# Borx25/CPU-Raytracing-experiments

Hardware: NVIDIA B200
Metric: Mrays/s (higher is better)
Workload: dtype f32

## Files before the change

__graft_entry__.py:

```python
import os
import subprocess
import sys

ROOT = os.path.dirname(os.path.abspath(__file__))
PKG = os.path.join(ROOT, "cpu-raytracing-experiments_b200")
CSRC = os.path.join(PKG, "csrc")
NVCC = os.environ.get("NVCC", "/usr/local/cuda/bin/nvcc")

NVCC_FLAGS = ["-gencode", "arch=compute_100a,code=sm_100a", "-lineinfo", "-O3", "-std=c++17", "-fmad=false",
              "-Xcompiler", "-fPIC,-ffp-contract=off,-O2", "-shared"]


def _newer(target, sources):
    if not os.path.exists(target):
        return True
    t = os.path.getmtime(target)
    return any(os.path.getmtime(s) > t for s in sources)


def build_lib(force=False):
    srcs = [os.path.join(CSRC, f) for f in ("b2r.cu", "b2r_host.cpp")]
    deps = srcs + [os.path.join(CSRC, f) for f in ("b2r_device.cuh", "b2r_shade.h", "b2r_math.h", "b2r_host.h")] + [os.path.join(ROOT, "include", "b2r.h")]
    out = os.path.join(PKG, "libb2r.so")
    if force or _newer(out, deps):
        subprocess.check_call([NVCC] + NVCC_FLAGS + srcs + ["-o", out])
    return out


def build_hostcheck(force=False):
    src = os.path.join(ROOT, "tests", "hostcheck", "hostcheck.cpp")
    out = os.path.join(ROOT, "tests", "hostcheck", "libhostcheck.so")
    cam = os.path.join(ROOT, "tests", "hostcheck", "mirror_camera.cpp")
    deps = [src, cam] + [os.path.join(CSRC, f) for f in ("b2r_host.cpp", "b2r_shade.h", "b2r_math.h", "b2r_host.h")] + [os.path.join(PKG, "host", f) for f in ("Camera.hpp", "Core.hpp")]
    if force or _newer(out, deps):
        subprocess.check_call(["g++", "-std=c++17", "-O2", "-ffp-contract=off", "-mavx2", "-mfma", "-fPIC", "-shared",
                               "-I/usr/local/cuda/include", "-I", CSRC, "-I", os.path.join(PKG, "host"), src, cam, os.path.join(CSRC, "b2r_host.cpp"), "-o", out])
    return out


def build_oracle():
    sys.path.insert(0, os.path.join(ROOT, "oracle"))
    import oracle_py
    srcs = [os.path.join(ROOT, "oracle", f) for f in ("oracle.cpp", "oracle_math.hpp")]
    force = any(_newer(os.path.join(ROOT, "oracle", n), srcs) for n in ("liboracle.so", "liboracle_fast.so"))
    oracle_py.build(force=force)


def build_refbinding(force=False):
    if not os.path.isdir("/root/reference"):
        return None
    d = os.path.join(ROOT, "tests", "refbinding"); out = os.path.join(d, "refbinding")
    deps = [os.path.join(d, "refbinding.cpp"), os.path.join(d, "build.sh"), os.path.join(ROOT, "include", "b2r_reference_binding.hpp"),
            os.path.join(ROOT, "include", "b2r.h"), os.path.join(PKG, "libb2r.so")]
    if force or _newer(out, deps):
        subprocess.check_call([os.path.join(d, "build.sh")], stdout=subprocess.DEVNULL)
    return out


def build():
    build_lib()
    build_oracle()
    build_hostcheck()
    build_refbinding()
    sys.path.insert(0, PKG)
    import b2r
    L = b2r.lib()
    assert L.b2r_abi_version() == 1
    missing = [s for s in b2r.ABI_SYMBOLS if not hasattr(L, s)]
    assert not missing, missing


def smoke():
    import numpy as np
    build()
    sys.path.insert(0, PKG); sys.path.insert(0, os.path.join(ROOT, "oracle"))
    import b2r, scenes, oracle_py
    W, H, MB, K = 256, 144, 8, 5
    sc = scenes.default_scene()
    r = b2r.Renderer(sc, W, H, max_bounces=MB, buckets=K)
    r.Accumulate(K)
    assert r.Render()
    o = oracle_py.Oracle(W, H, max_bounces=MB, K=K); o.set_scene(sc); o.accumulate(K)
    rc, ref = o.render()
    gb, ob = r.buckets_host(), o.buckets()
    rel = np.abs(gb - ob) / np.maximum(np.abs(ob), 1e-6)
    divergent = float((rel > 1e-4).any(axis=(0, 1)).mean())
    rmse = float(np.sqrt(np.mean((r.framebuffer[..., :3] - ref[..., :3]) ** 2)))
    print(f"smoke: brute default scene {W}x{H} K={K}: divergent pixel fraction {divergent:.2e}, bit-exact {bool((gb.view(np.uint32) == ob.view(np.uint32)).all())}, framebuffer RMSE {rmse:.3e}; counters {r.counters()}")
    assert divergent < 1e-3 and rmse < 1e-3
    if oracle_py.have_reference_renderer():
        rr = oracle_py.ReferenceRenderer(sc, W, H, MB); rr.accumulate(K); rb = rr.buckets(); _, rframe = rr.render(); rr.close()
        relr = np.abs(gb - rb) / np.maximum(np.abs(rb), 1e-6)
        div_r = float((relr > 1e-4).any(axis=(0, 1)).mean())
        rmse_r = float(np.sqrt(np.mean((r.framebuffer[..., :3] - rframe[..., :3]) ** 2)))
        print(f"smoke: against THE REFERENCE's Renderer::Accumulate/Render (oracle/_ref/librefrenderer.so): divergent pixel fraction {div_r:.2e}, framebuffer RMSE {rmse_r:.3e}")
        assert div_r < 5e-3 and rmse_r < 5e-3
    sc2 = scenes.random_scene(600, light_every=40)
    r2 = b2r.Renderer(sc2, 128, 64, max_bounces=6, buckets=1, flags=b2r.FLAG_FORCE_BVH)
    r2.Accumulate(2)
    o2 = oracle_py.Oracle(128, 64, max_bounces=6, K=1); o2.set_scene(sc2); o2.accumulate(2)
    g2, ob2 = r2.buckets_host(), o2.buckets()
    rel2 = np.abs(g2 - ob2) / np.maximum(np.abs(ob2), 1e-6)
    div2 = float((rel2 > 1e-4).any(axis=(0, 1)).mean())
    print(f"smoke: BVH pipeline random600 128x64: divergent pixel fraction {div2:.2e}")
    assert div2 < 5e-3
    geo = sc2["geometry"].copy(); rs = np.random.RandomState(1)
    geo["position"] += (rs.uniform(-0.5, 0.5, (len(geo), 3)) * np.sqrt(geo["radius_sq"])[:, None]).astype(np.float32)
    q = r2.RefitScene(geo); r2.ResetAccumulator(); r2.Accumulate(2)
    sc3 = scenes.Scene(sc2); sc3["geometry"] = geo
    o3 = oracle_py.Oracle(128, 64, max_bounces=6, K=1); o3.set_scene(sc3); o3.accumulate(2)
    g3, ob3 = r2.buckets_host(), o3.buckets()
    div3 = float(((np.abs(g3 - ob3) / np.maximum(np.abs(ob3), 1e-6)) > 1e-4).any(axis=(0, 1)).mean())
    print(f"smoke: after b2r_refit_scene (every sphere moved, tree quality ratio {q:.3f}): divergent pixel fraction {div3:.2e}")
    assert div3 < 5e-3
    r3 = b2r.Renderer(sc3, 128, 64, max_bounces=6, buckets=1, flags=b2r.FLAG_FORCE_BVH | b2r.FLAG_GPU_TREE | b2r.FLAG_GPU_SAH)
    r3.Accumulate(2)
    same = r3.buckets_host().tobytes() == g3.tobytes()
    print(f"smoke: device-built sweep tree ({len(r3.wide_nodes()[0])} wide nodes): buckets bit-identical to the host-built tree's: {same}")
    assert same
# ... 9 lines not shown
```

cpu-raytracing-experiments_b200/b2r.py:

```python
import ctypes as C
import os

import numpy as np

try:
    from . import scenes as _scenes
except ImportError:
    import scenes as _scenes

_HERE = os.path.dirname(os.path.abspath(__file__))
LIB_PATH = os.environ.get("B2R_LIB_PATH", os.path.join(_HERE, "libb2r.so"))

FLAG_FORCE_BRUTE, FLAG_FORCE_BVH, FLAG_NO_MIS, FLAG_COUNT_TESTS, FLAG_NO_GRAPH, FLAG_REFERENCE_TREE, FLAG_REFERENCE_EXACT, FLAG_NO_SPECULATION, FLAG_GPU_TREE = 1, 2, 4, 8, 16, 32, 64, 128, 256
FLAG_GPU_SAH = 1024
FLAG_GPU_SAH3 = 2048
FLAG_GGX = 512
FLAG_DIELECTRIC = 4096
TAP_CLOSEST, TAP_SHADOW, TAP_PACKET = 0, 1, 2
OK, ERR_ARG, ERR_CUDA, ERR_STATE, ERR_NO_LIGHTS, ERR_BVH, NOT_READY = 0, -1, -2, -3, -4, -5, 1
KERNEL_KINDS = ["generate", "bounce_brute", "intersect_closest", "shade", "intersect_shadow", "accumulate", "resolve"]
COUNTER_NAMES = ["extension_rays", "shadow_rays", "shaded_hits", "terminated", "dropped", "sphere_tests", "box_tests", "launches", "radiance_events", "reserved"]

ABI_SYMBOLS = [
    "b2r_bvh_build", "b2r_bvh_build_ex", "b2r_find_lights", "b2r_camera_lookat", "b2r_camera_ray", "b2r_create", "b2r_destroy", "b2r_resize", "b2r_reset", "b2r_set_stream",
    "b2r_sync", "b2r_upload_scene", "b2r_refit_scene", "b2r_set_camera", "b2r_set_lens", "b2r_accumulate", "b2r_resolve", "b2r_resolve_async", "b2r_resolve_device", "b2r_frame_wait", "b2r_resolve_from", "b2r_ipc_export_buckets", "b2r_ipc_open_peers", "b2r_ipc_close", "b2r_resolve_peers", "b2r_team_export", "b2r_team_open", "b2r_team_resolve", "b2r_team_error", "b2r_team_close", "b2r_host_register", "b2r_host_unregister", "b2r_get_accumulations", "b2r_set_accumulations",
    "b2r_read_buckets", "b2r_write_buckets", "b2r_save_checkpoint", "b2r_load_checkpoint", "b2r_device_buckets", "b2r_device_framebuffer", "b2r_read_counters", "b2r_reset_counters", "b2r_read_bounce_counts",
    "b2r_read_kernel_times", "b2r_set_flags", "b2r_generate_rays", "b2r_trace_closest", "b2r_trace_shadow", "b2r_trace_kernel", "b2r_read_wide_nodes", "b2r_read_link_tables", "b2r_get_origin_box",
    "b2r_write_hdr", "b2r_read_hdr", "b2r_last_error", "b2r_abi_version",
]


class B2RError(RuntimeError):
    def __init__(self, code, text):
        super().__init__(f"libb2r error {code}: {text}")
        self.code = code


class Config(C.Structure):
    _fields_ = [("width", C.c_uint32), ("height", C.c_uint32), ("max_bounces", C.c_uint32), ("buckets", C.c_uint32), ("flags", C.c_uint32),
                ("device", C.c_int32), ("bucket_first", C.c_uint32), ("bucket_stride", C.c_uint32), ("samples_in_flight", C.c_uint32)]


_lib = None


def lib():
    global _lib
    if _lib is None:
        if not os.path.exists(LIB_PATH):
            raise B2RError(ERR_STATE, f"{LIB_PATH} not built - run `python -c 'import __graft_entry__ as g; g.build()'`")
        L = C.CDLL(LIB_PATH)
        vp, u32, i32, f32 = C.c_void_p, C.c_uint32, C.c_int32, C.c_float
        sig = {
            "b2r_bvh_build": [vp, u32, vp, vp, vp, vp], "b2r_bvh_build_ex": [vp, u32, u32, f32, vp, vp, vp, vp], "b2r_find_lights": [vp, u32, vp, u32, vp, vp],
            "b2r_camera_lookat": [vp, vp, u32, u32, f32, f32, vp], "b2r_camera_ray": [vp, vp, f32, f32, f32, i32, i32, vp, vp, vp], "b2r_create": [vp, vp], "b2r_resize": [vp, u32, u32], "b2r_reset": [vp],
            "b2r_set_stream": [vp, vp], "b2r_sync": [vp],
            "b2r_upload_scene": [vp, vp, vp, u32, u32, vp, u32, vp, u32, vp, u32, vp, vp, i32, i32],
            "b2r_refit_scene": [vp, vp, u32, vp, u32, vp, u32, vp, u32, vp],
            "b2r_set_camera": [vp, vp, vp, f32, f32, f32, f32], "b2r_set_lens": [vp, f32, f32], "b2r_accumulate": [vp, u32], "b2r_resolve": [vp, vp, C.c_int], "b2r_resolve_async": [vp, vp, C.c_int], "b2r_resolve_device": [vp, C.c_int], "b2r_frame_wait": [vp], "b2r_resolve_from": [vp, vp, vp, C.c_int], "b2r_ipc_export_buckets": [vp, vp], "b2r_ipc_open_peers": [vp, vp, u32, u32], "b2r_ipc_close": [vp], "b2r_resolve_peers": [vp, vp, C.c_int], "b2r_team_export": [vp, vp], "b2r_team_open": [vp, vp, u32, u32], "b2r_team_resolve": [vp, vp, C.c_int, C.c_int], "b2r_team_error": [vp, vp], "b2r_team_close": [vp],
            "b2r_host_register": [vp, C.c_size_t], "b2r_host_unregister": [vp], "b2r_get_accumulations": [vp, vp], "b2r_set_accumulations": [vp, u32], "b2r_read_buckets": [vp, vp], "b2r_write_buckets": [vp, vp],
            "b2r_device_buckets": [vp, vp, vp], "b2r_device_framebuffer": [vp, vp, vp], "b2r_read_counters": [vp, vp], "b2r_reset_counters": [vp], "b2r_read_bounce_counts": [vp, vp, vp, u32],
            "b2r_read_kernel_times": [vp, vp, vp, C.c_int], "b2r_set_flags": [vp, u32], "b2r_generate_rays": [vp, u32, vp],
            "b2r_save_checkpoint": [vp, C.c_char_p], "b2r_load_checkpoint": [vp, C.c_char_p], "b2r_write_hdr": [C.c_char_p, vp, u32, u32], "b2r_read_hdr": [C.c_char_p, vp, vp, vp], "b2r_trace_closest": [vp, vp, u32, vp, vp], "b2r_trace_shadow": [vp, vp, vp, u32, vp], "b2r_trace_kernel": [vp, C.c_int, vp, vp, vp, vp, u32, u32, vp, vp, vp], "b2r_read_wide_nodes": [vp, vp, vp, vp], "b2r_read_link_tables": [vp, vp, vp], "b2r_get_origin_box": [vp, vp],
        }
        for name, args in sig.items():
            fn = getattr(L, name); fn.argtypes = args; fn.restype = C.c_int
        L.b2r_destroy.argtypes = [vp]; L.b2r_destroy.restype = None
        L.b2r_last_error.restype = C.c_char_p; L.b2r_abi_version.restype = C.c_int
        _lib = L
    return _lib


def _check(rc):
    if rc < 0:
        raise B2RError(rc, lib().b2r_last_error().decode())
    return rc


def _ptr(a):
    return C.c_void_p(a.ctypes.data) if a is not None else None


def build_bvh(geometry, log_cluster_size=0, cost_ratio=1.0):
    geo = np.ascontiguousarray(geometry, dtype=_scenes.SPHERE_DTYPE); n = len(geo)
    nodes = np.zeros(max(1, 2 * n - 1), _scenes.NODE_DTYPE); prims = np.zeros(n, _scenes.SPHERE_DTYPE); ids = np.zeros(n, np.uint32)
    nn = C.c_uint32(0)
    _check(lib().b2r_bvh_build_ex(_ptr(geo), n, log_cluster_size, cost_ratio, _ptr(nodes), _ptr(prims), _ptr(ids), C.addressof(nn)))
    return nodes[:nn.value], prims, ids


def find_lights(geometry, material):
    geo = np.ascontiguousarray(geometry, dtype=_scenes.SPHERE_DTYPE); mat = np.ascontiguousarray(material, dtype=_scenes.MATERIAL_DTYPE)
    out = np.zeros(len(geo), np.int32); n = C.c_uint32(0)
    _check(lib().b2r_find_lights(_ptr(geo), len(geo), _ptr(mat), len(mat), _ptr(out), C.addressof(n)))
    return out[:n.value].copy()


def camera_lookat(eye, direction, width, height, focal_length, exposure=1.0):
    out = np.zeros(11, np.float32)
    e = np.asarray(eye, np.float32); d = np.asarray(direction, np.float32)
    _check(lib().b2r_camera_lookat(_ptr(e), _ptr(d), width, height, focal_length, exposure, _ptr(out)))
    return out


class PreparedScene:

    def __init__(self, scene, width, height):
        self.scene = scene
        self.geometry = np.ascontiguousarray(scene["geometry"], dtype=_scenes.SPHERE_DTYPE)
        self.material = np.ascontiguousarray(scene["material"], dtype=_scenes.MATERIAL_DTYPE)
        self.nodes, self.prims, self.prim_ids = build_bvh(self.geometry)
        self.lights = find_lights(self.geometry, self.material)
        self.ambient = np.asarray(scene["ambient"], np.float32)
        self.hdri = None if scene.get("hdri") is None else np.ascontiguousarray(scene["hdri"], np.float32)
        self.set_view(width, height)

    def set_view(self, width, height):
        cam = self.scene["camera"]
        self.camera = camera_lookat(cam["eye"], cam["dir"], width, height, cam["focal_length"], cam["exposure"])


class Renderer:

    TileRoot = 16

    @staticmethod
    def RequiredTiling():
        return 16

    def __init__(self, scene, width, height, max_bounces=16, buckets=5, flags=0, device=0, bucket_first=0, bucket_stride=0,
                 samples_in_flight=0, stream=None):
        self._h = C.c_void_p(None)
        cfg = Config(width, height, max_bounces, buckets, flags, device, bucket_first, bucket_stride, samples_in_flight)
        _check(lib().b2r_create(C.byref(self._h), C.byref(cfg)))
        self.width, self.height, self.max_bounces, self.buckets, self.flags = width, height, max_bounces, buckets, flags
        self.h_tiles, self.v_tiles = width // 16, height // 16
        self.framebuffer = np.zeros((height, width, 4), np.float32)
        if stream is not None:
            _check(lib().b2r_set_stream(self._h, C.c_void_p(stream)))
        self.scene = None
        if scene is not None:
            self.SetScene(scene)

    def close(self):
        if getattr(self, "_h", None) and self._h.value:
            lib().b2r_destroy(self._h); self._h = C.c_void_p(None)
# ... 101 lines not shown
        return _check(lib().b2r_team_resolve(self._h, _ptr(dst), 1 if tonemap else 0, 1 if use_async else 0)) == OK

    def team_error(self):
        v = C.c_uint32(0); _check(lib().b2r_team_error(self._h, C.byref(v))); return v.value

    def GetFrame(self):
        return self.framebuffer

    def sync(self):
        _check(lib().b2r_sync(self._h))

    def buckets_host(self):
        out = np.empty((self.buckets, 3, self.width * self.height), np.float32); _check(lib().b2r_read_buckets(self._h, _ptr(out))); return out

    def write_buckets(self, arr):
        a = np.ascontiguousarray(arr, np.float32); _check(lib().b2r_write_buckets(self._h, _ptr(a)))

    def SaveCheckpoint(self, path):
        _check(lib().b2r_save_checkpoint(self._h, str(path).encode()))

    def LoadCheckpoint(self, path):
        _check(lib().b2r_load_checkpoint(self._h, str(path).encode()))

    def device_buckets(self):
        p = C.c_void_p(None); n = C.c_size_t(0); _check(lib().b2r_device_buckets(self._h, C.byref(p), C.byref(n))); return p.value, n.value

    def device_framebuffer(self):
        p = C.c_void_p(None); n = C.c_size_t(0); _check(lib().b2r_device_framebuffer(self._h, C.byref(p), C.byref(n))); return p.value, n.value

    def counters(self):
        out = (C.c_uint64 * 10)(); _check(lib().b2r_read_counters(self._h, out)); return dict(zip(COUNTER_NAMES, out[:]))

    def bounce_counts(self):
        n = self.max_bounces + 1; a = np.zeros(n, np.uint32); b = np.zeros(n, np.uint32)
        _check(lib().b2r_read_bounce_counts(self._h, _ptr(a), _ptr(b), n)); return a, b

    def reset_counters(self):
        _check(lib().b2r_reset_counters(self._h))

    def kernel_times(self, reset=True):
        ms = (C.c_double * 8)(); n = (C.c_uint64 * 8)(); _check(lib().b2r_read_kernel_times(self._h, ms, n, 1 if reset else 0))
        return {k: (ms[i], n[i]) for i, k in enumerate(KERNEL_KINDS)}

    def set_flags(self, flags):
        _check(lib().b2r_set_flags(self._h, flags)); self.flags = flags

    def generate_rays(self, acc):
        out = np.empty((self.width * self.height, 6), np.float32); _check(lib().b2r_generate_rays(self._h, acc, _ptr(out))); return out

    def trace_closest(self, rays):
        r = np.ascontiguousarray(rays, np.float32); n = len(r); t = np.empty(n, np.float32); p = np.empty(n, np.int32)
        _check(lib().b2r_trace_closest(self._h, _ptr(r), n, _ptr(t), _ptr(p))); return t, p

    def trace_shadow(self, rays, tfar):
        r = np.ascontiguousarray(rays, np.float32); tf = np.ascontiguousarray(tfar, np.float32); n = len(r); o = np.empty(n, np.uint8)
        _check(lib().b2r_trace_shadow(self._h, _ptr(r), _ptr(tf), n, _ptr(o))); return o

    def trace_kernel_closest(self, rays, tail=None):
        r = np.ascontiguousarray(rays, np.float32); n = len(r); t = np.empty(n, np.float32); p = np.empty(n, np.int32)
        tl = None if tail is None else np.ascontiguousarray(tail, np.uint8)
        _check(lib().b2r_trace_kernel(self._h, TAP_CLOSEST, _ptr(r), None, None, _ptr(tl), n, 0, _ptr(t), _ptr(p), None)); return t, p

    def trace_kernel_shadow(self, rays, tfar, origin_prim):
        r = np.ascontiguousarray(rays, np.float32); tf = np.ascontiguousarray(tfar, np.float32); op = np.ascontiguousarray(origin_prim, np.int32)
        n = len(r); o = np.empty(n, np.uint8)
        _check(lib().b2r_trace_kernel(self._h, TAP_SHADOW, _ptr(r), _ptr(tf), _ptr(op), None, n, 0, None, None, _ptr(o))); return o

    def trace_kernel_packet(self, acc):
        n = self.width * self.height; t = np.empty(n, np.float32); p = np.empty(n, np.int32)
        _check(lib().b2r_trace_kernel(self._h, TAP_PACKET, None, None, None, None, n, acc, _ptr(t), _ptr(p), None)); return t, p

    def link_tables(self):
        n = C.c_uint32(0); _check(lib().b2r_read_wide_nodes(self._h, None, C.byref(n), None))
        parent = np.empty(n.value, np.uint32); leaf = np.empty(len(self.scene.prims), np.uint32)
        _check(lib().b2r_read_link_tables(self._h, _ptr(parent), _ptr(leaf))); return parent, leaf

    def wide_nodes(self):
        n = C.c_uint32(0); ms = C.c_uint32(0)
        _check(lib().b2r_read_wide_nodes(self._h, None, C.byref(n), C.byref(ms)))
        out = np.zeros((n.value, 4, 8), np.float32)
        _check(lib().b2r_read_wide_nodes(self._h, _ptr(out), C.byref(n), C.byref(ms)))
        return out, ms.value

    def origin_box(self):
        out = np.zeros(6, np.float32); _check(lib().b2r_get_origin_box(self._h, _ptr(out))); return out


def host_register(arr):
    _check(lib().b2r_host_register(_ptr(arr), arr.nbytes))


def host_unregister(arr):
    _check(lib().b2r_host_unregister(_ptr(arr)))


def write_hdr(path, rgba):
    a = np.ascontiguousarray(rgba, np.float32)
    _check(lib().b2r_write_hdr(str(path).encode(), _ptr(a), a.shape[1], a.shape[0]))


def read_hdr(path):
    w, h = C.c_int32(0), C.c_int32(0)
    if lib().b2r_read_hdr(str(path).encode(), None, C.byref(w), C.byref(h)) != OK:
        raise B2RError(ERR_ARG, f"{path}: not a Radiance .hdr stb_image would load")
    out = np.empty((h.value, w.value, 4), np.float32)
    if lib().b2r_read_hdr(str(path).encode(), _ptr(out), C.byref(w), C.byref(h)) != OK:
        raise B2RError(ERR_ARG, f"{path}: corrupt or truncated .hdr")
    return out


def tile_to_raster(buf, width, height):
    ht, vt = width // 16, height // 16
    a = np.asarray(buf).reshape(buf.shape[:-1] + (vt, ht, 16, 16))
    return np.moveaxis(a, -2, -3).reshape(buf.shape[:-1] + (height, width))
```

cpu-raytracing-experiments_b200/csrc/b2r.cu:

```cuda
#include "b2r_device.cuh"

#include <cub/device/device_radix_sort.cuh>
#include <cub/device/device_scan.cuh>

#include <algorithm>
#include <cstdio>
#include <cstdlib>
#include <cstring>
#include <string>
#include <vector>

using namespace b2r;

namespace {

thread_local std::string g_error;
int fail(int code, const std::string& what) { g_error = what; return code; }
constexpr const char* kDielInvalid = "B2R_FLAG_DIELECTRIC: a material has a non-finite transmission, or is dielectric (max(transmission) > 0) with a transmission outside [0, 1] or 1 + IOR_minus_one not finite or < 1";
#define CU(expr) do { cudaError_t e_ = (expr); if (e_ != cudaSuccess) return fail(B2R_ERR_CUDA, std::string(#expr) + ": " + cudaGetErrorString(e_)); } while (0)

enum KernelKind { KK_GENERATE = 0, KK_BRUTE, KK_CLOSEST, KK_SHADE, KK_SHADOW, KK_ACCUMULATE, KK_RESOLVE, KK_COUNT };

constexpr uint32_t kMaxLanes = 4;
struct BatchArgs {
	uint32_t n; uint32_t acc[kMaxSlots]; unsigned long long fold = ~0ull; CameraParams cam; LensParams lens{0.0f, 0.0f};
	uint32_t lanes = 0, lane_slots = 0, n_lane[kMaxLanes] = {0, 0, 0, 0};
	uint32_t slot_of(uint32_t i) const {
		if (lanes == 0u) return i;
		uint32_t j = 0; while (j + 1u < lanes && i >= n_lane[j]) { i -= n_lane[j]; j++; }
		return j * lane_slots + i;
	}
};
__global__ void k_set_batch(BatchDev* dst, const BatchArgs a) {
	if (threadIdx.x == 0) { dst[0].n_slots = a.n; dst[0].fold = a.fold; dst[0].cam = a.cam; dst[0].lens = a.lens; }
	if (threadIdx.x < a.n) dst[0].acc[threadIdx.x] = a.acc[threadIdx.x];
	for (uint32_t j = 0; j < kMaxLanes; j++) {
		const uint32_t nj = j < a.lanes ? a.n_lane[j] : 0u;
		if (threadIdx.x == 0) { dst[1 + j].n_slots = nj; dst[1 + j].fold = 0ull; dst[1 + j].cam = a.cam; dst[1 + j].lens = a.lens; }
		if (threadIdx.x < nj) dst[1 + j].acc[threadIdx.x] = a.acc[j * a.lane_slots + threadIdx.x];
	}
}

template <typename T> int dev_alloc(T** p, size_t count) {
	if (*p) { cudaFree(*p); *p = nullptr; }
	if (count == 0) count = 1;
	CU(cudaMalloc(reinterpret_cast<void**>(p), count * sizeof(T)));
	return B2R_OK;
}
template <typename T> int dev_reserve(T** p, size_t* capacity, size_t count) {
	if (count == 0) count = 1;
	if (*p && *capacity >= count) return B2R_OK;
	if (*p) { cudaFree(*p); *p = nullptr; *capacity = 0; }
	CU(cudaMalloc(reinterpret_cast<void**>(p), count * sizeof(T)));
	*capacity = count;
	return B2R_OK;
}
template <typename T> void dev_free(T** p) { if (*p) { cudaFree(*p); *p = nullptr; } }

#define B2R_PACKED_TABLES(X) X(float4, prims, LEN_PRIMS) X(int32_t, prim_mat, LEN_PRIMS) X(float4, mat_albedo, LEN_MAT) X(float4, mat_emission, LEN_MAT) \
                             X(float4, mat_f0, LEN_MAT) X(float4, mat_diel, LEN_MAT) X(float4, light_sphere, LEN_LIGHTS) X(float4, light_emit, LEN_LIGHTS)
#define B2R_SCENE_TABLES(X) B2R_PACKED_TABLES(X) X(WideNode, wide, LEN_WIDE) X(uint32_t, parent, LEN_WIDE) X(uint32_t, leaf_node, LEN_PRIMS) X(float4, hdri, LEN_TEXELS)
enum TableLen { LEN_PRIMS = 0, LEN_MAT, LEN_LIGHTS, LEN_WIDE, LEN_TEXELS, LEN_COUNT };
struct SceneTables {
	template <typename T> struct Table { T* p = nullptr; size_t cap = 0; };
#define X(T, name, len) Table<T> name;
	B2R_SCENE_TABLES(X)
#undef X
	template <typename F, typename... S> static int for_each(F&& f, S&... sets) {
		int rc = B2R_OK;
#define X(T, name, len) if (rc == B2R_OK) rc = f(len, sets.name...);
		B2R_SCENE_TABLES(X)
#undef X
		return rc;
	}
};
void free_tables(SceneTables& t) { SceneTables::for_each([](int, auto& x) -> int { dev_free(&x.p); x.cap = 0; return B2R_OK; }, t); }
void bind_tables(Params& p, const SceneTables& t, bool sky) {
	SceneDev& s = p.scene;
	s.prims = t.prims.p; s.prim_mat = t.prim_mat.p; s.mat_albedo = t.mat_albedo.p; s.mat_emission = t.mat_emission.p; s.mat_f0 = t.mat_f0.p;
	s.light_sphere = t.light_sphere.p; s.light_emit = t.light_emit.p; s.wide = t.wide.p; s.parent = t.parent.p; s.leaf_node = t.leaf_node.p;
	s.hdri = sky ? t.hdri.p : nullptr;
	p.mat_diel = t.mat_diel.p;
}

}

struct b2r_ctx {
	b2r_config cfg{};
	cudaStream_t stream = nullptr, own_stream = nullptr;
	unsigned char* h_stage = nullptr; size_t stage_bytes = 0; cudaEvent_t ev_stage = nullptr; bool stage_busy = false;
	cudaStream_t copy_stream = nullptr; cudaEvent_t ev_resolved = nullptr, ev_copied = nullptr; bool copy_pending = false;
	bool have_scene = false, have_camera = false, use_bvh = false;
	uint32_t accumulations = 0;
	uint32_t slots = 8;
	int sm_count = 0;
	SceneTables tables;
	bool scene_diel_valid = true;
	WideBvh wide_host; uint64_t wide_key = 0; std::vector<unsigned char> wide_blob; bool have_wide = false;
	uint32_t n_wide = 0;
	bool gpu_tree = false; uint32_t *d_mkey[2] = {nullptr, nullptr}, *d_midx[2] = {nullptr, nullptr}; size_t cap_mkey = 0; uint8_t* d_sort_tmp = nullptr; size_t cap_sort_tmp = 0; uint8_t* d_sweep = nullptr; size_t cap_sweep = 0;
	std::vector<b2r_sphere> lazy_prims, lazy_geom; double* d_cost_base = nullptr;
	std::vector<uint32_t> cur_geom_of_prim;
	uint32_t* d_remap = nullptr; size_t cap_remap = 0;
	uint8_t* d_trace = nullptr; size_t cap_trace = 0;
	uint8_t* d_tap = nullptr; size_t cap_tap = 0;
	bool wide_refit = false; double* d_cost = nullptr;
	OriginBox obox{}; bool obox_valid = false; float sph_lo[3] = {0, 0, 0}, sph_hi[3] = {0, 0, 0}; float cam_pos[3] = {0, 0, 0};
	LensParams lens{0.0f, 0.0f};
	float4 *d_A[2] = {nullptr, nullptr}, *d_B[2] = {nullptr, nullptr}, *d_SA = nullptr, *d_SB = nullptr, *d_fb = nullptr;
	float *d_T[2] = {nullptr, nullptr}, *d_SL = nullptr, *d_rad = nullptr, *d_acc = nullptr;
	uint8_t *d_ex_slot[2] = {nullptr, nullptr}, *d_ex_key = nullptr; uint16_t* d_ex_act[2] = {nullptr, nullptr}; uint32_t* d_ex_next = nullptr;
	float2* d_H = nullptr; uint32_t* d_SS = nullptr;
	uint32_t* d_counts = nullptr; size_t counts_bytes = 0;
	unsigned long long* d_stats = nullptr;
	BatchDev* d_batch = nullptr;
	Params params{};
	int grid_brute_first_exact = 0, grid_brute_exact = 0;
	int grid_brute_first_ggx = 0, grid_brute_ggx = 0, grid_brute_finish_ggx = 0, grid_shade_ggx = 0;
	int grid_brute_first = 0, grid_brute = 0, grid_closest = 0, grid_shade = 0, grid_shadow = 0, grid_stream = 0, grid_packet = 0, grid_brute_finish = 0; bool packet_primary = true;
	int grid_brute_first_lens = 0, grid_brute_first_ggx_lens = 0, grid_packet_lens = 0;
	int grid_diel_brute_first[2][2] = {{0, 0}, {0, 0}}, grid_diel_brute[2] = {0, 0}, grid_diel_finish[2] = {0, 0}, grid_diel_shade[2] = {0, 0};
	cudaGraphExec_t graph_exec = nullptr; bool graph_valid = false;
	cudaGraphExec_t lane_exec[kMaxLanes + 1] = {nullptr, nullptr, nullptr, nullptr, nullptr}; bool lane_valid[kMaxLanes + 1] = {false, false, false, false, false};
	bool idle = true;
	uint32_t lanes_max = 2; bool lanes_forced = false;
	cudaStream_t lane_stream[kMaxLanes] = {nullptr, nullptr, nullptr, nullptr}; cudaEvent_t ev_fork = nullptr, ev_join[kMaxLanes] = {nullptr, nullptr, nullptr, nullptr};
	float lane_grid_frac = 1.0f;
	uint64_t graph_launches = 0, lane_launches[kMaxLanes + 1] = {0, 0, 0, 0, 0};
	struct Side {
		cudaStream_t stream = nullptr, lane_stream[kMaxLanes] = {nullptr, nullptr, nullptr, nullptr};
		cudaEvent_t ev_traced = nullptr, ev_folded = nullptr, ev_sync = nullptr, ev_fork = nullptr, ev_join[kMaxLanes] = {nullptr, nullptr, nullptr, nullptr};
		bool folded_valid = false; uint64_t epoch = ~0ull;
		SceneTables tables;
		bool have_copy = false, refreshed_valid = false; uint64_t scene_version = ~0ull; cudaEvent_t ev_refreshed = nullptr;
		cudaGraphExec_t exec[kMaxLanes + 1] = {nullptr, nullptr, nullptr, nullptr, nullptr}; bool valid[kMaxLanes + 1] = {false, false, false, false, false}; uint64_t launches[kMaxLanes + 1] = {0, 0, 0, 0, 0};
	} side[2];
	uint32_t sides = 2, next_side = 0, last_side = 0, spec_side = 0, counts_first = 0;
	uint64_t scene_epoch = 0;
	cudaStream_t up_stream = nullptr, scene_st = nullptr; cudaEvent_t ev_uploaded = nullptr, ev_main_mark = nullptr; bool uploaded_valid = false;
	uint64_t scene_version = 0;
	bool main_reads_scene = false;
	size_t hdri_texels = 0;
	uint64_t launches = 0;
	struct Timed { int kind; cudaEvent_t a, b; };
	std::vector<Timed> timed;
	double kernel_ms[8] = {0}; uint64_t kernel_launches[8] = {0};
	std::vector<void*> peer_acc; uint32_t my_rank = 0;
	uint32_t spec_width = 1, spec_first = 0, spec_count = 0, spec_used = 0; BatchArgs spec_args;
	TeamSync* d_team = nullptr; std::vector<void*> team_acc, team_sync; void* team_fb0 = nullptr; uint32_t team_rank = 0, team_frame = 0; bool team_wait_done = false;
};

namespace {

int ensure_device(b2r_ctx* c) { CU(cudaSetDevice(c->cfg.device)); return B2R_OK; }
cudaError_t sync_main(b2r_ctx* c) { c->idle = true; return cudaStreamSynchronize(c->stream); }
constexpr uint32_t kSpecMax = 16;
constexpr uint32_t kFinishBelow = 12000000u;
void drop_speculation(b2r_ctx* c) { c->spec_count = 0; c->spec_used = 0; c->spec_width = 1; }

void drop_graph(b2r_ctx* c) {
	drop_speculation(c);
	if (c->stream) sync_main(c);
	if (c->graph_exec) { cudaGraphExecDestroy(c->graph_exec); c->graph_exec = nullptr; }
	for (uint32_t l = 0; l <= kMaxLanes; l++) { if (c->lane_exec[l]) { cudaGraphExecDestroy(c->lane_exec[l]); c->lane_exec[l] = nullptr; } c->lane_valid[l] = false; }
	for (auto& S : c->side) {
		if (S.stream) cudaStreamSynchronize(S.stream);
		for (uint32_t l = 0; l <= kMaxLanes; l++) { if (S.exec[l]) { cudaGraphExecDestroy(S.exec[l]); S.exec[l] = nullptr; } S.valid[l] = false; }
	}
	c->graph_valid = false;
}

int alloc_frame(b2r_ctx* c) {
	const uint32_t w = c->cfg.width, h = c->cfg.height, npix = w * h, mb = c->cfg.max_bounces, K = c->cfg.buckets;
	if (c->cfg.samples_in_flight == 0) {
		uint32_t s = (128u << 20) / npix; c->slots = s < 4u ? 4u : s > static_cast<uint32_t>(kMaxSlots) ? static_cast<uint32_t>(kMaxSlots) : s;
	}
	const size_t cap = static_cast<size_t>(c->slots) * npix;
	if (3 * cap >= (1ull << 32)) return fail(B2R_ERR_ARG, "samples_in_flight * pixels too large: the three-plane queue arrays are indexed with 32 bits");
	int rc;
	for (int s = 0; s < 2; s++) {
		if ((rc = dev_alloc(&c->d_A[s], cap))) return rc;
		if ((rc = dev_alloc(&c->d_B[s], cap))) return rc;
		if ((rc = dev_alloc(&c->d_T[s], 3 * cap))) return rc;
	}
	if ((rc = dev_alloc(&c->d_H, cap))) return rc;
	if ((rc = dev_alloc(&c->d_SA, cap))) return rc;
	if ((rc = dev_alloc(&c->d_SB, cap))) return rc;
	if ((rc = dev_alloc(&c->d_SL, 3 * cap))) return rc;
	if ((rc = dev_alloc(&c->d_SS, cap))) return rc;
	if ((rc = dev_alloc(&c->d_rad, 3 * cap))) return rc;
	if ((rc = dev_alloc(&c->d_acc, static_cast<size_t>(K) * 3 * npix))) return rc;
	if ((rc = dev_alloc(&c->d_fb, static_cast<size_t>(npix)))) return rc;
	c->counts_bytes = (static_cast<size_t>(mb) + 1) * 4 * sizeof(uint32_t);
	if ((rc = dev_alloc(&c->d_counts, (static_cast<size_t>(mb) + 1) * 4 * kMaxLanes * 2))) return rc;
	CU(cudaMemset(c->d_counts, 0, 2 * kMaxLanes * c->counts_bytes));
	if (!c->d_stats) { if ((rc = dev_alloc(&c->d_stats, static_cast<size_t>(ST_COUNT)))) return rc; CU(cudaMemset(c->d_stats, 0, ST_COUNT * sizeof(unsigned long long))); }
	if (!c->d_batch) { if ((rc = dev_alloc(&c->d_batch, static_cast<size_t>(2 * (1 + kMaxLanes))))) return rc; }
	if (c->cfg.flags & B2R_FLAG_REFERENCE_EXACT) {
		for (int s = 0; s < 2; s++) { if ((rc = dev_alloc(&c->d_ex_slot[s], cap))) return rc; if ((rc = dev_alloc(&c->d_ex_act[s], cap / 256))) return rc; }
		if ((rc = dev_alloc(&c->d_ex_key, cap))) return rc;
		if ((rc = dev_alloc(&c->d_ex_next, cap))) return rc;
		CU(cudaMemset(c->d_ex_key, 0, cap));
	}
	CU(cudaMemset(c->d_rad, 0, 3 * cap * sizeof(float)));
	CU(cudaMemset(c->d_acc, 0, static_cast<size_t>(K) * 3 * npix * sizeof(float)));
	Params& p = c->params;
	p.frame.width = w; p.frame.height = h; p.frame.h_tiles = w / 16; p.frame.npix = npix;
	p.frame.h_tiles_magic = magic_for(w / 16); p.frame.npix_magic = magic_for(npix);
	p.frame.max_bounces = mb; p.frame.buckets = K; p.frame.flags = c->cfg.flags;
	{
		const char* e = std::getenv("B2R_FINISH_BELOW"); const char* f = std::getenv("B2R_FINISH_FIRST");
		p.frame.finish_below = e ? static_cast<uint32_t>(std::strtoul(e, nullptr, 10)) : kFinishBelow;
		p.frame.finish_first = f ? static_cast<uint32_t>(std::strtoul(f, nullptr, 10)) : 2u;
	}
	for (int s = 0; s < 2; s++) { p.q.A[s] = c->d_A[s]; p.q.B[s] = c->d_B[s]; p.q.T[s] = c->d_T[s]; }
	p.q.H = c->d_H; p.q.SA = c->d_SA; p.q.SB = c->d_SB; p.q.SL = c->d_SL; p.q.SS = c->d_SS; p.q.cap = static_cast<uint32_t>(cap);
	p.cnt.paths = c->d_counts; p.cnt.shadow = c->d_counts + (mb + 1); p.cnt.work_a = c->d_counts + 2 * (mb + 1); p.cnt.work_b = c->d_counts + 3 * (mb + 1);
	p.cnt.stats = c->d_stats;
	p.batch = c->d_batch; p.rad = c->d_rad; p.acc = c->d_acc;
	for (int s = 0; s < 2; s++) { p.ex.slot[s] = c->d_ex_slot[s]; p.ex.act[s] = c->d_ex_act[s]; }
	p.ex.key = c->d_ex_key; p.ex.next_idx = c->d_ex_next;
	c->accumulations = 0;
	drop_graph(c);
	return B2R_OK;
}

int compute_grids(b2r_ctx* c) {
	auto occ = [&](const void* fn, int block, int* out) -> int {
		int n = 0; CU(cudaOccupancyMaxActiveBlocksPerMultiprocessor(&n, fn, block, 0));
		*out = (n < 1 ? 1 : n) * c->sm_count; return B2R_OK;
	};
	int rc;
	if ((rc = occ(reinterpret_cast<const void*>(&k_bounce_brute<true, false, false>), kBruteBlock, &c->grid_brute_first))) return rc;
	if ((rc = occ(reinterpret_cast<const void*>(&k_bounce_brute<false, false, false>), kBruteBlock, &c->grid_brute))) return rc;
	if ((rc = occ(reinterpret_cast<const void*>(&k_bounce_brute<true, false, true>), kBruteBlock, &c->grid_brute_first_exact))) return rc;
	if ((rc = occ(reinterpret_cast<const void*>(&k_bounce_brute<false, false, true>), kBruteBlock, &c->grid_brute_exact))) return rc;
	if ((rc = occ(reinterpret_cast<const void*>(&k_intersect_closest<false, false, 16u>), kTravBlock, &c->grid_closest))) return rc;
	if ((rc = occ(reinterpret_cast<const void*>(&k_shade<false>), kBruteBlock, &c->grid_shade))) return rc;
	if ((rc = occ(reinterpret_cast<const void*>(&k_intersect_shadow<false>), kTravBlock, &c->grid_shadow))) return rc;
	if ((rc = occ(reinterpret_cast<const void*>(&k_intersect_packet<false, B2R_PACKET_RPL>), kTravBlock, &c->grid_packet))) return rc;
	if ((rc = occ(reinterpret_cast<const void*>(&k_brute_finish<false>), kBruteBlock, &c->grid_brute_finish))) return rc;
	if ((rc = occ(reinterpret_cast<const void*>(&k_bounce_brute<true, false, false, true>), kBruteBlock, &c->grid_brute_first_ggx))) return rc;
	if ((rc = occ(reinterpret_cast<const void*>(&k_bounce_brute<false, false, false, true>), kBruteBlock, &c->grid_brute_ggx))) return rc;
	if ((rc = occ(reinterpret_cast<const void*>(&k_brute_finish<false, true>), kBruteBlock, &c->grid_brute_finish_ggx))) return rc;
	if ((rc = occ(reinterpret_cast<const void*>(&k_shade<false, true>), kBruteBlock, &c->grid_shade_ggx))) return rc;
	if ((rc = occ(reinterpret_cast<const void*>(&k_bounce_brute<true, false, false, false, true>), kBruteBlock, &c->grid_brute_first_lens))) return rc;
	if ((rc = occ(reinterpret_cast<const void*>(&k_bounce_brute<true, false, false, true, true>), kBruteBlock, &c->grid_brute_first_ggx_lens))) return rc;
	if ((rc = occ(reinterpret_cast<const void*>(&k_intersect_packet<false, B2R_PACKET_RPL_LENS, true>), kTravBlock, &c->grid_packet_lens))) return rc;
	const void* diel_first[2][2] = {{reinterpret_cast<const void*>(&k_bounce_brute<true, false, false, false, false, true>), reinterpret_cast<const void*>(&k_bounce_brute<true, false, false, false, true, true>)},
	                                {reinterpret_cast<const void*>(&k_bounce_brute<true, false, false, true, false, true>), reinterpret_cast<const void*>(&k_bounce_brute<true, false, false, true, true, true>)}};
	const void* diel_brute[2] = {reinterpret_cast<const void*>(&k_bounce_brute<false, false, false, false, false, true>), reinterpret_cast<const void*>(&k_bounce_brute<false, false, false, true, false, true>)};
	const void* diel_finish[2] = {reinterpret_cast<const void*>(&k_brute_finish<false, false, true>), reinterpret_cast<const void*>(&k_brute_finish<false, true, true>)};
	const void* diel_shade[2] = {reinterpret_cast<const void*>(&k_shade<false, false, true>), reinterpret_cast<const void*>(&k_shade<false, true, true>)};
	for (int g = 0; g < 2; g++) {
		for (int l = 0; l < 2; l++) if ((rc = occ(diel_first[g][l], kBruteBlock, &c->grid_diel_brute_first[g][l]))) return rc;
		if ((rc = occ(diel_brute[g], kBruteBlock, &c->grid_diel_brute[g])) || (rc = occ(diel_finish[g], kBruteBlock, &c->grid_diel_finish[g])) || (rc = occ(diel_shade[g], kBruteBlock, &c->grid_diel_shade[g]))) return rc;
	}
	c->packet_primary = std::getenv("B2R_NO_PACKET") == nullptr;
	c->lanes_max = std::getenv("B2R_NO_TWIN") ? 1u : 2u;
	if (const char* e = std::getenv("B2R_SIDES")) { c->sides = std::atoi(e) == 1 ? 1u : 2u; }
	if (const char* e = std::getenv("B2R_LANES")) { const int v = std::atoi(e); if (v == 1 || v == 2 || v == 4) { c->lanes_max = static_cast<uint32_t>(v); c->lanes_forced = true; } }
	if (const char* e = std::getenv("B2R_LANE_GRID")) { c->lane_grid_frac = static_cast<float>(std::atof(e)); if (!(c->lane_grid_frac > 0.0f && c->lane_grid_frac <= 1.0f)) c->lane_grid_frac = 1.0f; }
	c->grid_stream = c->sm_count * 8;
	return B2R_OK;
}

template <typename F> int launch(b2r_ctx* c, int kind, bool profile, F&& f) {
	b2r_ctx::Timed t{kind, nullptr, nullptr};
	if (profile) { CU(cudaEventCreate(&t.a)); CU(cudaEventCreate(&t.b)); CU(cudaEventRecord(t.a, c->stream)); }
	f();
	CU(cudaGetLastError());
	if (profile) { CU(cudaEventRecord(t.b, c->stream)); c->timed.push_back(t); }
	c->launches++;
	return B2R_OK;
}

using BounceKernel = void (*)(const Params, const uint32_t);
struct KernelSet {
	BounceKernel brute_first, brute, brute_finish, packet, closest, shade, shadow;
	void (*generate)(const Params);
	int g_brute_first, g_brute, g_brute_finish, g_packet, g_shade;
};
KernelSet pick_kernels(const b2r_ctx* c) {
	const bool count = (c->cfg.flags & B2R_FLAG_COUNT_TESTS) != 0, exact = (c->cfg.flags & B2R_FLAG_REFERENCE_EXACT) != 0, ggx = (c->cfg.flags & B2R_FLAG_GGX) != 0;
	const bool tn16 = c->params.scene.stack_tn_bits == 16u;
	const bool lens = c->lens.radius > 0.0f && !exact;
	const bool diel = (c->cfg.flags & B2R_FLAG_DIELECTRIC) != 0;
	KernelSet k{};
	if (ggx)        { k.brute_first = k_bounce_brute<true, false, false, true>; k.brute = k_bounce_brute<false, false, false, true>; k.g_brute_first = c->grid_brute_first_ggx; k.g_brute = c->grid_brute_ggx; }
	else if (exact) { k.brute_first = count ? k_bounce_brute<true, true, true> : k_bounce_brute<true, false, true>; k.brute = count ? k_bounce_brute<false, true, true> : k_bounce_brute<false, false, true>; k.g_brute_first = c->grid_brute_first_exact; k.g_brute = c->grid_brute_exact; }
	else            { k.brute_first = count ? k_bounce_brute<true, true, false> : k_bounce_brute<true, false, false>; k.brute = count ? k_bounce_brute<false, true, false> : k_bounce_brute<false, false, false>; k.g_brute_first = c->grid_brute_first; k.g_brute = c->grid_brute; }
	if (lens && ggx) { k.brute_first = k_bounce_brute<true, false, false, true, true>; k.g_brute_first = c->grid_brute_first_ggx_lens; }
	else if (lens)   { k.brute_first = count ? k_bounce_brute<true, true, false, false, true> : k_bounce_brute<true, false, false, false, true>; k.g_brute_first = c->grid_brute_first_lens; }
	k.brute_finish = ggx ? k_brute_finish<false, true> : count ? k_brute_finish<true> : k_brute_finish<false>;
	k.g_brute_finish = ggx ? c->grid_brute_finish_ggx : c->grid_brute_finish;
	if (lens) { k.packet = count ? k_intersect_packet<true, B2R_PACKET_RPL_LENS, true> : k_intersect_packet<false, B2R_PACKET_RPL_LENS, true>; k.g_packet = c->grid_packet_lens; }
	else      { k.packet = count ? k_intersect_packet<true, B2R_PACKET_RPL> : k_intersect_packet<false, B2R_PACKET_RPL>; k.g_packet = c->grid_packet; }
	k.generate = lens ? k_generate<true> : k_generate<false>;
	if (exact) k.closest = count ? (tn16 ? k_intersect_closest<true, true, 16u> : k_intersect_closest<true, true, 0u>) : (tn16 ? k_intersect_closest<false, true, 16u> : k_intersect_closest<false, true, 0u>);
	else       k.closest = count ? (tn16 ? k_intersect_closest<true, false, 16u> : k_intersect_closest<true, false, 0u>) : (tn16 ? k_intersect_closest<false, false, 16u> : k_intersect_closest<false, false, 0u>);
	k.shade = ggx ? k_shade<false, true> : exact ? k_shade<true> : k_shade<false>;
	k.g_shade = ggx ? c->grid_shade_ggx : c->grid_shade;
	if (diel) {
		const int g = ggx ? 1 : 0, l = lens ? 1 : 0;
		if (ggx) {
			k.brute_first = lens ? k_bounce_brute<true, false, false, true, true, true> : k_bounce_brute<true, false, false, true, false, true>;
			k.brute = k_bounce_brute<false, false, false, true, false, true>; k.brute_finish = k_brute_finish<false, true, true>; k.shade = k_shade<false, true, true>;
		} else {
			k.brute_first = lens ? k_bounce_brute<true, false, false, false, true, true> : k_bounce_brute<true, false, false, false, false, true>;
			k.brute = k_bounce_brute<false, false, false, false, false, true>; k.brute_finish = k_brute_finish<false, false, true>; k.shade = k_shade<false, false, true>;
		}
		k.g_brute_first = c->grid_diel_brute_first[g][l]; k.g_brute = c->grid_diel_brute[g]; k.g_brute_finish = c->grid_diel_finish[g]; k.g_shade = c->grid_diel_shade[g];
	}
	k.shadow = count ? k_intersect_shadow<true> : k_intersect_shadow<false>;
	return k;
}

int enqueue_rounds(b2r_ctx* c, const Params& p_in, cudaStream_t st, bool profile, float grid_frac = 1.0f, uint32_t lanes = 1) {
	auto G = [&](int g) { const int per_sm = g / c->sm_count; int k = static_cast<int>(per_sm * grid_frac + 0.5f); if (k < 1) k = 1; return k * c->sm_count; };
	const bool exact = (c->cfg.flags & B2R_FLAG_REFERENCE_EXACT) != 0;
	if (exact && c->params.scene.n_mat > 64) return fail(B2R_ERR_STATE, "B2R_FLAG_REFERENCE_EXACT: at most 64 materials (RendererPolicy::max_materialID, Renderer.hpp:23)");
	const KernelSet k = pick_kernels(c);
	const uint32_t mb = c->cfg.max_bounces;
	Params p = p_in;
	int rc;
	auto run = [&](int kind, BounceKernel fn, int grid, int block, uint32_t b) { return launch(c, kind, profile, [&] { fn<<<grid, block, 0, st>>>(p, b); }); };
	if (!c->use_bvh) {
		const bool finish = !exact && p.frame.finish_below != 0u && p.scene.n_prims <= static_cast<uint32_t>(kBruteTile);
		if (!finish) p.frame.finish_below = 0u;
		else if (lanes > 1u) p.frame.finish_below /= lanes;
		for (uint32_t b = 0; b < mb; b++) {
			if (finish && b >= p.frame.finish_first && b + 1 < mb && (rc = run(KK_BRUTE, k.brute_finish, k.g_brute_finish, kBruteBlock, b))) return rc;
			if ((rc = b == 0 ? run(KK_BRUTE, k.brute_first, k.g_brute_first, kBruteBlock, b) : run(KK_BRUTE, k.brute, k.g_brute, kBruteBlock, b))) return rc;
			if (exact && b + 1 < mb && (rc = run(KK_BRUTE, k_stream_rank, c->grid_stream, 256, b))) return rc;
		}
		return B2R_OK;
	}
	if (!c->packet_primary && (rc = launch(c, KK_GENERATE, profile, [&] { k.generate<<<c->grid_stream, kBlock, 0, st>>>(p); }))) return rc;
	const bool mis = !(c->cfg.flags & B2R_FLAG_NO_MIS);
	for (uint32_t b = 0; b < mb; b++) {
		if (b == 0 && c->packet_primary) { if ((rc = run(KK_CLOSEST, k.packet, G(k.g_packet), kTravBlock, b))) return rc; }
		else if ((rc = run(KK_CLOSEST, k.closest, G(c->grid_closest), kTravBlock, b))) return rc;
		if ((rc = run(KK_SHADE, k.shade, G(k.g_shade), kBruteBlock, b))) return rc;
		if (exact && b + 1 < mb && (rc = run(KK_SHADE, k_stream_rank, c->grid_stream, 256, b))) return rc;
		if (mis && b + 1 < mb && (rc = run(KK_SHADOW, k.shadow, G(c->grid_shadow), kTravBlock, b))) return rc;
	}
	return B2R_OK;
}

bool sides_for(const b2r_ctx* c, bool use_bvh) { return c->sides == 2u && use_bvh && !(c->cfg.flags & (B2R_FLAG_NO_GRAPH | B2R_FLAG_REFERENCE_EXACT)) && c->slots >= 2u && c->slots % 2u == 0u; }
bool use_sides(const b2r_ctx* c) { return sides_for(c, c->use_bvh); }
uint32_t batch_cap(const b2r_ctx* c) { return use_sides(c) ? c->slots / 2u : c->slots; }
uint32_t lane_slots_of(const b2r_ctx* c, uint32_t lanes) { return (batch_cap(c) + lanes - 1u) / lanes; }
Params lane_params(const b2r_ctx* c, uint32_t which, uint32_t lanes, uint32_t side = 0) {
	Params p = c->params;
	const uint32_t cap_slots = batch_cap(c), ls = lane_slots_of(c, lanes), rel = which * ls, mine = rel >= cap_slots ? 0u : (cap_slots - rel < ls ? cap_slots - rel : ls);
	const size_t npix = p.frame.npix, off = static_cast<size_t>(side * cap_slots + rel) * npix, cap = static_cast<size_t>(mine) * npix;
	for (int s = 0; s < 2; s++) { p.q.A[s] += off; p.q.B[s] += off; p.q.T[s] += 3 * off; }
	p.q.H += off; p.q.SA += off; p.q.SB += off; p.q.SL += 3 * off; p.q.SS += off; p.q.cap = static_cast<uint32_t>(cap);
	const uint32_t block = (c->cfg.max_bounces + 1u) * 4u, blk = side * kMaxLanes + which;
	p.cnt.paths += blk * block; p.cnt.shadow += blk * block; p.cnt.work_a += blk * block; p.cnt.work_b += blk * block;
	p.batch = c->d_batch + side * (1u + kMaxLanes) + 1u + which;
	p.rad += 3 * off;
	if (use_sides(c)) bind_tables(p, c->side[side].tables, p.scene.hdri != nullptr);
	return p;
}
Params side_params(const b2r_ctx* c, uint32_t side) {
	Params p = c->params;
	p.batch = c->d_batch + side * (1u + kMaxLanes);
	p.rad += 3 * static_cast<size_t>(side * batch_cap(c)) * p.frame.npix;
	return p;
}
int enqueue_trace(b2r_ctx* c, uint32_t sidx, uint32_t lanes) {
	b2r_ctx::Side& S = c->side[sidx];
	cudaStream_t st = S.stream;
	CU(cudaMemsetAsync(c->d_counts + static_cast<size_t>(sidx) * kMaxLanes * (c->counts_bytes / sizeof(uint32_t)), 0, kMaxLanes * c->counts_bytes, st));
	int rc;
	if (lanes <= 1u) { Params p = lane_params(c, 0, 1, sidx); p.batch = c->d_batch + sidx * (1u + kMaxLanes); return enqueue_rounds(c, p, st, false); }
	CU(cudaEventRecord(S.ev_fork, st));
	for (uint32_t j = 1; j < lanes; j++) CU(cudaStreamWaitEvent(S.lane_stream[j], S.ev_fork, 0));
	for (uint32_t j = 0; j < lanes; j++) if ((rc = enqueue_rounds(c, lane_params(c, j, lanes, sidx), j ? S.lane_stream[j] : st, false, c->lane_grid_frac, lanes))) return rc;
	for (uint32_t j = 1; j < lanes; j++) { CU(cudaEventRecord(S.ev_join[j], S.lane_stream[j])); CU(cudaStreamWaitEvent(st, S.ev_join[j], 0)); }
	return B2R_OK;
}

int enqueue_batch(b2r_ctx* c, bool profile, uint32_t lanes) {
	cudaStream_t st = c->stream;
	CU(cudaMemsetAsync(c->d_counts, 0, kMaxLanes * c->counts_bytes, st));
	int rc;
	if (lanes <= 1u) { if ((rc = enqueue_rounds(c, c->params, st, profile))) return rc; }
	else {
		CU(cudaEventRecord(c->ev_fork, st));
		for (uint32_t j = 1; j < lanes; j++) CU(cudaStreamWaitEvent(c->lane_stream[j], c->ev_fork, 0));
		for (uint32_t j = 0; j < lanes; j++) if ((rc = enqueue_rounds(c, lane_params(c, j, lanes), j ? c->lane_stream[j] : st, false, c->lane_grid_frac, lanes))) return rc;
		for (uint32_t j = 1; j < lanes; j++) { CU(cudaEventRecord(c->ev_join[j], c->lane_stream[j])); CU(cudaStreamWaitEvent(st, c->ev_join[j], 0)); }
	}
	return launch(c, KK_ACCUMULATE, profile, [&] { k_accumulate<<<c->grid_stream, kBlock, 0, st>>>(c->params); });
}

int refresh_side_scene(b2r_ctx* c, uint32_t sidx);
int run_batch(b2r_ctx* c, BatchArgs& args) {
	const bool no_graph = (c->cfg.flags & B2R_FLAG_NO_GRAPH) != 0;
	uint32_t lanes = 1;
	if (!no_graph && !(c->cfg.flags & B2R_FLAG_REFERENCE_EXACT)) {
		if (c->lanes_max >= 4u && args.n >= 4u && batch_cap(c) % 4u == 0u) lanes = 4;
		else if (c->lanes_max >= 2u && args.n >= 2u && batch_cap(c) >= 2u) lanes = 2;
		if (use_sides(c) && !c->lanes_forced && !c->idle && c->side[c->next_side].epoch == c->scene_epoch) lanes = 1;
	}
	c->idle = false;
	if (lanes > 1u) {
		const uint32_t n = args.n, ls = lane_slots_of(c, lanes);
		uint32_t acc[kMaxSlots]; for (uint32_t i = 0; i < n; i++) acc[i] = args.acc[i];
		unsigned long long fold = 0ull; uint32_t i = 0, span = 0;
		for (uint32_t s = 0; s < static_cast<uint32_t>(kMaxSlots); s++) args.acc[s] = 0u;
		for (uint32_t j = 0; j < lanes; j++) {
			const uint32_t nj = n / lanes + (j < n % lanes ? 1u : 0u);
			args.n_lane[j] = nj;
			for (uint32_t k = 0; k < nj; k++, i++) { const uint32_t slot = j * ls + k; args.acc[slot] = acc[i]; if ((args.fold >> i) & 1ull) fold |= 1ull << slot; if (slot + 1u > span) span = slot + 1u; }
		}
		args.lanes = lanes; args.lane_slots = ls; args.n = span; args.fold = fold;
	} else { args.lanes = 0; args.lane_slots = 0; if (args.n < 64u) args.fold &= (1ull << args.n) - 1ull; }
	args.cam = c->params.frame.cam; args.lens = c->lens;
	if (use_sides(c)) {
		const uint32_t sidx = c->next_side; c->next_side ^= 1u;
		b2r_ctx::Side& S = c->side[sidx];
		if (!S.stream) {
			CU(cudaStreamCreateWithFlags(&S.stream, cudaStreamNonBlocking));
			for (cudaEvent_t* e : {&S.ev_traced, &S.ev_folded, &S.ev_sync, &S.ev_fork}) CU(cudaEventCreateWithFlags(e, cudaEventDisableTiming));
		}
		for (uint32_t j = 1; j < lanes; j++) if (!S.lane_stream[j]) { CU(cudaStreamCreateWithFlags(&S.lane_stream[j], cudaStreamNonBlocking)); CU(cudaEventCreateWithFlags(&S.ev_join[j], cudaEventDisableTiming)); }
		if (S.epoch != c->scene_epoch) { CU(cudaEventRecord(S.ev_sync, c->stream)); CU(cudaStreamWaitEvent(S.stream, S.ev_sync, 0)); S.epoch = c->scene_epoch; }
		if (S.folded_valid) CU(cudaStreamWaitEvent(S.stream, S.ev_folded, 0));
		{ const int rc = refresh_side_scene(c, sidx); if (rc) return rc; }
		k_set_batch<<<1, kMaxSlots, 0, S.stream>>>(c->d_batch + sidx * (1u + kMaxLanes), args);
		CU(cudaGetLastError());
		if (!S.valid[lanes]) {
			if (S.exec[lanes]) { CU(cudaStreamSynchronize(S.stream)); cudaGraphExecDestroy(S.exec[lanes]); S.exec[lanes] = nullptr; }
			cudaGraph_t graph = nullptr;
			const uint64_t before = c->launches;
			CU(cudaStreamBeginCapture(S.stream, cudaStreamCaptureModeThreadLocal));
			int rc = enqueue_trace(c, sidx, lanes);
			cudaError_t e = cudaStreamEndCapture(S.stream, &graph);
// ... 221 lines not shown
		const uint32_t first = lf[l], count = lf[l + 1] - lf[l];
		k_refit_level<<<(count * 4u + kBlock - 1u) / kBlock, kBlock, 0, c->scene_st>>>(reinterpret_cast<float4*>(c->tables.wide.p), c->tables.prims.p, d_remap, c->obox, first, count);
		c->launches++;
	}
	CU(cudaGetLastError());
	return B2R_OK;
}
int launch_link_tables(b2r_ctx* c) {
	k_link_tables<<<(c->n_wide * 4u + kBlock - 1u) / kBlock, kBlock, 0, c->scene_st>>>(reinterpret_cast<const float4*>(c->tables.wide.p), c->n_wide, c->tables.parent.p, c->tables.leaf_node.p);
	CU(cudaGetLastError()); c->launches++;
	return B2R_OK;
}
uint32_t camera_origins(const b2r_ctx* c, float out[6]) {
	if (!c->have_camera) return 0u;
	const float r = c->lens.radius;
	if (r == 0.0f) { for (int k = 0; k < 3; k++) out[k] = c->cam_pos[k]; return 1u; }
	for (int k = 0; k < 3; k++) { out[k] = c->cam_pos[k] - r; out[3 + k] = c->cam_pos[k] + r; }
	return 2u;
}
int ensure_origin_box(b2r_ctx* c, const float* points, uint32_t n_points) {
	if (c->obox_valid && origin_box_holds(c->obox, points, n_points)) return B2R_OK;
	std::vector<float> extra(points, points + 3 * static_cast<size_t>(n_points));
	float cam[6]; const uint32_t n_cam = camera_origins(c, cam);
	extra.insert(extra.end(), cam, cam + 3 * n_cam);
	if (c->obox_valid) { extra.insert(extra.end(), c->obox.lo, c->obox.lo + 3); extra.insert(extra.end(), c->obox.hi, c->obox.hi + 3); }
	c->obox = origin_box_rule(c->sph_lo, c->sph_hi, extra.data(), static_cast<uint32_t>(extra.size() / 3)); c->obox_valid = true;
	if (c->have_wide && !c->gpu_tree) wide_fill_boxes(c->wide_host, c->wide_host.prims.data(), c->obox);
	if (c->have_scene && c->have_wide) {
		int rc = begin_scene_write(c, use_sides(c)); if (rc) return rc;
		if ((rc = launch_refit_levels(c, nullptr))) return rc;
		return end_scene_write(c);
	}
	return B2R_OK;
}

}

extern "C" {

static int team_before_bucket_write(b2r_ctx* c);
const char* b2r_last_error(void) { return g_error.c_str(); }
int b2r_abi_version(void) { return B2R_ABI_VERSION; }

int b2r_create(b2r_ctx** out, const b2r_config* cfg) {
	if (!out || !cfg) return fail(B2R_ERR_ARG, "null argument");
	*out = nullptr;
	if (cfg->width == 0 || cfg->height == 0 || cfg->width % 16 || cfg->height % 16) return fail(B2R_ERR_ARG, "width/height must be non-zero multiples of 16 (Renderer::RequiredTiling)");
	if (static_cast<uint64_t>(cfg->width) * cfg->height > kPixMask) return fail(B2R_ERR_ARG, "image too large (2^26 pixels max)");
	if (cfg->buckets < 1 || cfg->buckets > 64) return fail(B2R_ERR_ARG, "buckets must be in 1..64");
	if (cfg->max_bounces < 1 || cfg->max_bounces > 1024) return fail(B2R_ERR_ARG, "max_bounces must be in 1..1024");
	if (cfg->bucket_stride > 1 && cfg->bucket_first >= cfg->bucket_stride) return fail(B2R_ERR_ARG, "bucket_first must be < bucket_stride");
	if (cfg->samples_in_flight > static_cast<uint32_t>(kMaxSlots)) return fail(B2R_ERR_ARG, "samples_in_flight must be <= 64");
	if ((cfg->flags & B2R_FLAG_GGX) && (cfg->flags & B2R_FLAG_REFERENCE_EXACT)) return fail(B2R_ERR_ARG, "B2R_FLAG_GGX cannot be combined with B2R_FLAG_REFERENCE_EXACT");
	if ((cfg->flags & B2R_FLAG_DIELECTRIC) && (cfg->flags & B2R_FLAG_REFERENCE_EXACT)) return fail(B2R_ERR_ARG, "B2R_FLAG_DIELECTRIC cannot be combined with B2R_FLAG_REFERENCE_EXACT");
	int n_dev = 0;
	cudaError_t e = cudaGetDeviceCount(&n_dev);
	if (e != cudaSuccess || n_dev == 0) return fail(B2R_ERR_CUDA, std::string("no CUDA device: ") + cudaGetErrorString(e) + " (libb2r has no CPU fallback)");
	if (cfg->device < 0 || cfg->device >= n_dev) return fail(B2R_ERR_ARG, "device ordinal out of range");
	b2r_ctx* c = new b2r_ctx();
	c->cfg = *cfg;
	c->slots = cfg->samples_in_flight;
	int rc = ensure_device(c);
	if (!rc) { cudaDeviceProp prop; e = cudaGetDeviceProperties(&prop, cfg->device); if (e != cudaSuccess) rc = fail(B2R_ERR_CUDA, cudaGetErrorString(e)); else c->sm_count = prop.multiProcessorCount; }
	if (!rc) { e = cudaStreamCreateWithFlags(&c->own_stream, cudaStreamNonBlocking); if (e != cudaSuccess) rc = fail(B2R_ERR_CUDA, cudaGetErrorString(e)); c->stream = c->own_stream; }
	if (!rc) rc = compute_grids(c);
	if (!rc) rc = alloc_frame(c);
	if (rc) { b2r_destroy(c); return rc; }
	*out = c;
	return B2R_OK;
}

void b2r_destroy(b2r_ctx* c) {
	if (!c) return;
	cudaSetDevice(c->cfg.device);
	if (c->stream) sync_main(c);
	for (size_t r = 0; r < c->peer_acc.size(); r++) if (c->peer_acc[r] && r != c->my_rank) cudaIpcCloseMemHandle(c->peer_acc[r]);
	b2r_team_close(c); if (c->d_team) { cudaFree(c->d_team); c->d_team = nullptr; }
	drop_graph(c);
	for (auto& t : c->timed) { cudaEventDestroy(t.a); cudaEventDestroy(t.b); }
	free_tables(c->tables);
	dev_free(&c->d_cost); dev_free(&c->d_remap); dev_free(&c->d_trace); dev_free(&c->d_tap); dev_free(&c->d_cost_base); dev_free(&c->d_sort_tmp); dev_free(&c->d_sweep);
	for (int k = 0; k < 2; k++) { dev_free(&c->d_mkey[k]); dev_free(&c->d_midx[k]); }
	for (int s = 0; s < 2; s++) { dev_free(&c->d_A[s]); dev_free(&c->d_B[s]); dev_free(&c->d_T[s]); }
	dev_free(&c->d_H); dev_free(&c->d_SA); dev_free(&c->d_SB); dev_free(&c->d_SL); dev_free(&c->d_SS); dev_free(&c->d_rad); dev_free(&c->d_acc); dev_free(&c->d_fb);
	for (int s = 0; s < 2; s++) { dev_free(&c->d_ex_slot[s]); dev_free(&c->d_ex_act[s]); }
	dev_free(&c->d_ex_key); dev_free(&c->d_ex_next);
	dev_free(&c->d_counts); dev_free(&c->d_stats); dev_free(&c->d_batch);
	if (c->h_stage) cudaFreeHost(c->h_stage);
	if (c->ev_stage) cudaEventDestroy(c->ev_stage);
	if (c->copy_stream) { cudaStreamSynchronize(c->copy_stream); cudaStreamDestroy(c->copy_stream); cudaEventDestroy(c->ev_resolved); cudaEventDestroy(c->ev_copied); }
	free_side_scenes(c);
	if (c->up_stream) { cudaStreamSynchronize(c->up_stream); cudaStreamDestroy(c->up_stream); cudaEventDestroy(c->ev_main_mark); }
	if (c->ev_uploaded) cudaEventDestroy(c->ev_uploaded);
	for (auto& S : c->side) {
		if (S.ev_refreshed) cudaEventDestroy(S.ev_refreshed);
		for (uint32_t j = 1; j < kMaxLanes; j++) if (S.lane_stream[j]) { cudaStreamDestroy(S.lane_stream[j]); cudaEventDestroy(S.ev_join[j]); }
		if (S.stream) { cudaStreamDestroy(S.stream); cudaEventDestroy(S.ev_traced); cudaEventDestroy(S.ev_folded); cudaEventDestroy(S.ev_sync); cudaEventDestroy(S.ev_fork); }
	}
	for (uint32_t j = 1; j < kMaxLanes; j++) if (c->lane_stream[j]) { cudaStreamDestroy(c->lane_stream[j]); cudaEventDestroy(c->ev_join[j]); }
	if (c->ev_fork) cudaEventDestroy(c->ev_fork);
	if (c->own_stream) cudaStreamDestroy(c->own_stream);
	delete c;
}

int b2r_resize(b2r_ctx* c, uint32_t width, uint32_t height) {
	if (!c) return fail(B2R_ERR_ARG, "null context");
	if (width == 0 || height == 0 || width % 16 || height % 16) return fail(B2R_ERR_ARG, "width/height must be non-zero multiples of 16");
	if (static_cast<uint64_t>(width) * height > kPixMask) return fail(B2R_ERR_ARG, "image too large");
	int rc = ensure_device(c); if (rc) return rc;
	CU(sync_main(c));
	if (c->copy_pending) { CU(cudaEventSynchronize(c->ev_copied)); c->copy_pending = false; }
	if (width == c->cfg.width && height == c->cfg.height) return b2r_reset(c);
	if (!c->peer_acc.empty() || !c->team_acc.empty()) return fail(B2R_ERR_STATE, "the bucket array / framebuffer are exported to peers (CUDA IPC): b2r_ipc_close / b2r_team_close on every rank before a resize, then export again");
	c->cfg.width = width; c->cfg.height = height;
	return alloc_frame(c);
}

int b2r_reset(b2r_ctx* c) {
	if (!c) return fail(B2R_ERR_ARG, "null context");
	int rc = ensure_device(c); if (rc) return rc;
	c->accumulations = 0; drop_speculation(c);
	if ((rc = team_before_bucket_write(c))) return rc;
	const size_t npix = static_cast<size_t>(c->cfg.width) * c->cfg.height;
	CU(cudaMemsetAsync(c->d_acc, 0, static_cast<size_t>(c->cfg.buckets) * 3 * npix * sizeof(float), c->stream));
	return B2R_OK;
}

int b2r_set_stream(b2r_ctx* c, void* cuda_stream) {
	if (!c) return fail(B2R_ERR_ARG, "null context");
	int rc = ensure_device(c); if (rc) return rc;
	CU(sync_main(c));
	c->stream = cuda_stream ? static_cast<cudaStream_t>(cuda_stream) : c->own_stream;
	drop_graph(c);
	return B2R_OK;
}

int b2r_sync(b2r_ctx* c) {
	if (!c) return fail(B2R_ERR_ARG, "null context");
	int rc = ensure_device(c); if (rc) return rc;
	CU(sync_main(c));
	return collect_timings(c);
}

int b2r_set_flags(b2r_ctx* c, uint32_t flags) {
	if (!c) return fail(B2R_ERR_ARG, "null context");
	int rc = ensure_device(c); if (rc) return rc;
	CU(sync_main(c));
	if ((c->cfg.flags ^ flags) & B2R_FLAG_REFERENCE_TREE) return fail(B2R_ERR_STATE, "B2R_FLAG_REFERENCE_TREE can only be chosen at b2r_create");
	if ((c->cfg.flags ^ flags) & B2R_FLAG_REFERENCE_EXACT) return fail(B2R_ERR_STATE, "B2R_FLAG_REFERENCE_EXACT can only be chosen at b2r_create");
	if ((flags & B2R_FLAG_GGX) && (flags & B2R_FLAG_REFERENCE_EXACT)) return fail(B2R_ERR_ARG, "B2R_FLAG_GGX cannot be combined with B2R_FLAG_REFERENCE_EXACT");
	if ((flags & B2R_FLAG_DIELECTRIC) && (flags & B2R_FLAG_REFERENCE_EXACT)) return fail(B2R_ERR_ARG, "B2R_FLAG_DIELECTRIC cannot be combined with B2R_FLAG_REFERENCE_EXACT");
	if ((flags & B2R_FLAG_DIELECTRIC) && c->have_scene && !c->scene_diel_valid) return fail(B2R_ERR_ARG, kDielInvalid);
	c->cfg.flags = flags; c->params.frame.flags = flags;
	if (c->have_scene) {
		const uint32_t n = c->params.scene.n_prims;
		c->use_bvh = (flags & B2R_FLAG_FORCE_BVH) ? true : (flags & B2R_FLAG_FORCE_BRUTE) ? false : n > 32;
	}
	drop_graph(c);
	return B2R_OK;
}

}
namespace {
struct UploadPart { void* dst; const void* src; size_t bytes; };
int stage_upload(b2r_ctx* c, const UploadPart* parts, size_t n_parts) {
	size_t total = 0; for (size_t i = 0; i < n_parts; i++) total += (parts[i].bytes + 255) & ~static_cast<size_t>(255);
	if (c->stage_busy) { CU(cudaEventSynchronize(c->ev_stage)); c->stage_busy = false; }
// ... 491 lines not shown
	return B2R_OK;
}
int b2r_host_unregister(void* ptr) {
	if (!ptr) return fail(B2R_ERR_ARG, "null argument");
	cudaError_t e = cudaHostUnregister(ptr);
	if (e != cudaSuccess) { cudaGetLastError(); return fail(B2R_ERR_CUDA, std::string("cudaHostUnregister: ") + cudaGetErrorString(e)); }
	return B2R_OK;
}
int b2r_get_accumulations(b2r_ctx* c, uint32_t* out) { if (!c || !out) return fail(B2R_ERR_ARG, "null argument"); *out = c->accumulations; return B2R_OK; }
int b2r_set_accumulations(b2r_ctx* c, uint32_t acc) { if (!c) return fail(B2R_ERR_ARG, "null context"); c->accumulations = acc; drop_speculation(c); return B2R_OK; }

int b2r_read_buckets(b2r_ctx* c, float* out_host) {
	if (!c || !out_host) return fail(B2R_ERR_ARG, "null argument");
	int rc = ensure_device(c); if (rc) return rc;
	CU(cudaMemcpyAsync(out_host, c->d_acc, static_cast<size_t>(c->cfg.buckets) * 3 * c->params.frame.npix * sizeof(float), cudaMemcpyDeviceToHost, c->stream));
	CU(sync_main(c));
	return collect_timings(c);
}
int b2r_write_buckets(b2r_ctx* c, const float* in_host) {
	if (!c || !in_host) return fail(B2R_ERR_ARG, "null argument");
	int rc = ensure_device(c); if (rc) return rc;
	drop_speculation(c);
	CU(cudaMemcpyAsync(c->d_acc, in_host, static_cast<size_t>(c->cfg.buckets) * 3 * c->params.frame.npix * sizeof(float), cudaMemcpyHostToDevice, c->stream));
	CU(sync_main(c));
	return B2R_OK;
}

namespace {
struct CheckpointHeader { char magic[8]; uint32_t width, height, buckets, max_bounces, accumulations, result_flags; uint64_t payload_hash; uint64_t payload_bytes; uint32_t reserved[4]; };
static_assert(sizeof(CheckpointHeader) == 64, "checkpoint header");
constexpr uint32_t kResultFlags = B2R_FLAG_NO_MIS | B2R_FLAG_REFERENCE_EXACT | B2R_FLAG_DIELECTRIC;
uint64_t fnv1a64(const void* data, size_t bytes) { const unsigned char* b = static_cast<const unsigned char*>(data); uint64_t h = 1469598103934665603ull; for (size_t i = 0; i < bytes; i++) h = (h ^ b[i]) * 1099511628211ull; return h; }
}
int b2r_save_checkpoint(b2r_ctx* c, const char* path) {
	if (!c || !path) return fail(B2R_ERR_ARG, "null argument");
	const size_t n = static_cast<size_t>(c->cfg.buckets) * 3 * c->params.frame.npix;
	std::vector<float> host(n);
	int rc = b2r_read_buckets(c, host.data()); if (rc) return rc;
	CheckpointHeader h{}; std::memcpy(h.magic, "B2RBUCK1", 8);
	h.width = c->cfg.width; h.height = c->cfg.height; h.buckets = c->cfg.buckets; h.max_bounces = c->cfg.max_bounces; h.accumulations = c->accumulations;
	h.result_flags = c->cfg.flags & kResultFlags; h.payload_bytes = n * sizeof(float); h.payload_hash = fnv1a64(host.data(), n * sizeof(float));
	FILE* f = std::fopen(path, "wb");
	if (!f) return fail(B2R_ERR_ARG, std::string("cannot open ") + path + " for writing");
	const bool ok = std::fwrite(&h, sizeof h, 1, f) == 1 && std::fwrite(host.data(), sizeof(float), n, f) == n;
	if (std::fclose(f) != 0 || !ok) return fail(B2R_ERR_ARG, std::string("short write to ") + path);
	return B2R_OK;
}
int b2r_load_checkpoint(b2r_ctx* c, const char* path) {
	if (!c || !path) return fail(B2R_ERR_ARG, "null argument");
	FILE* f = std::fopen(path, "rb");
	if (!f) return fail(B2R_ERR_ARG, std::string("cannot open ") + path);
	CheckpointHeader h{};
	const size_t n = static_cast<size_t>(c->cfg.buckets) * 3 * c->params.frame.npix;
	std::vector<float> host(n);
	bool ok = std::fread(&h, sizeof h, 1, f) == 1 && std::memcmp(h.magic, "B2RBUCK1", 8) == 0;
	const bool same = ok && h.width == c->cfg.width && h.height == c->cfg.height && h.buckets == c->cfg.buckets && h.max_bounces == c->cfg.max_bounces &&
	                  h.result_flags == (c->cfg.flags & kResultFlags) && h.payload_bytes == n * sizeof(float);
	if (same) ok = std::fread(host.data(), sizeof(float), n, f) == n && std::fgetc(f) == EOF && fnv1a64(host.data(), n * sizeof(float)) == h.payload_hash;
	std::fclose(f);
	if (!ok) return fail(B2R_ERR_ARG, std::string(path) + ": not a bucket checkpoint, truncated, or its payload hash does not match");
	if (!same) return fail(B2R_ERR_STATE, std::string(path) + ": written for another frame size, bucket count, bounce limit (the pixel seeds depend on width and max_bounces, Q2) or MIS / reference-exact mode");
	int rc = b2r_write_buckets(c, host.data()); if (rc) return rc;
	return b2r_set_accumulations(c, h.accumulations);
}

int b2r_device_buckets(b2r_ctx* c, void** dev_ptr, size_t* bytes) {
	if (!c || !dev_ptr || !bytes) return fail(B2R_ERR_ARG, "null argument");
	*dev_ptr = c->d_acc; *bytes = static_cast<size_t>(c->cfg.buckets) * 3 * c->params.frame.npix * sizeof(float);
	return B2R_OK;
}
int b2r_device_framebuffer(b2r_ctx* c, void** dev_ptr, size_t* bytes) {
	if (!c || !dev_ptr || !bytes) return fail(B2R_ERR_ARG, "null argument");
	*dev_ptr = c->d_fb; *bytes = static_cast<size_t>(c->params.frame.npix) * sizeof(float4);
	return B2R_OK;
}

int b2r_read_counters(b2r_ctx* c, uint64_t out[10]) {
	if (!c || !out) return fail(B2R_ERR_ARG, "null argument");
	int rc = ensure_device(c); if (rc) return rc;
	unsigned long long h[ST_COUNT];
	CU(cudaMemcpyAsync(h, c->d_stats, sizeof h, cudaMemcpyDeviceToHost, c->stream));
	CU(sync_main(c));
	out[0] = h[ST_EXT]; out[1] = h[ST_SHADOW]; out[2] = h[ST_HITS]; out[3] = h[ST_TERM]; out[4] = h[ST_DROPPED]; out[5] = h[ST_SPHERE]; out[6] = h[ST_BOX];
	out[7] = c->launches; out[8] = h[ST_EVENTS]; out[9] = 0;
	return collect_timings(c);
}
int b2r_read_bounce_counts(b2r_ctx* c, uint32_t* paths_out, uint32_t* shadow_out, uint32_t n) {
	if (!c || !paths_out || !shadow_out) return fail(B2R_ERR_ARG, "null argument");
	int rc = ensure_device(c); if (rc) return rc;
	const uint32_t mb = c->cfg.max_bounces;
	const size_t block = (static_cast<size_t>(mb) + 1) * 4;
	std::vector<uint32_t> h(block * kMaxLanes);
	CU(cudaMemcpyAsync(h.data(), c->d_counts + static_cast<size_t>(c->counts_first) * block, kMaxLanes * c->counts_bytes, cudaMemcpyDeviceToHost, c->stream));
	CU(sync_main(c));
	for (uint32_t b = 0; b < n; b++) {
		paths_out[b] = 0u; shadow_out[b] = 0u;
		for (uint32_t j = 0; j < kMaxLanes; j++) { if (b <= mb) paths_out[b] += h[j * block + b]; if (b < mb) shadow_out[b] += h[j * block + mb + 1 + b]; }
	}
	return collect_timings(c);
}
int b2r_reset_counters(b2r_ctx* c) {
	if (!c) return fail(B2R_ERR_ARG, "null context");
	int rc = ensure_device(c); if (rc) return rc;
	CU(cudaMemsetAsync(c->d_stats, 0, ST_COUNT * sizeof(unsigned long long), c->stream));
	c->launches = 0; c->scene_epoch++;
	return B2R_OK;
}
int b2r_read_kernel_times(b2r_ctx* c, double ms_out[8], uint64_t launches_out[8], int reset) {
	if (!c || !ms_out || !launches_out) return fail(B2R_ERR_ARG, "null argument");
	int rc = ensure_device(c); if (rc) return rc;
	if ((rc = collect_timings(c))) return rc;
	for (int i = 0; i < 8; i++) { ms_out[i] = c->kernel_ms[i]; launches_out[i] = c->kernel_launches[i]; if (reset) { c->kernel_ms[i] = 0; c->kernel_launches[i] = 0; } }
	return B2R_OK;
}

int b2r_generate_rays(b2r_ctx* c, uint32_t acc, float* out_host) {
	if (!c || !out_host) return fail(B2R_ERR_ARG, "null argument");
	if (!c->have_camera) return fail(B2R_ERR_STATE, "set_camera first");
	int rc = ensure_device(c); if (rc) return rc;
	float* d = nullptr; const size_t n = static_cast<size_t>(c->params.frame.npix) * 6;
	if ((rc = dev_alloc(&d, n))) return rc;
	if (c->lens.radius > 0.0f) k_tap_generate<true><<<c->grid_stream, kBlock, 0, c->stream>>>(c->params, acc, c->lens, d);
	else k_tap_generate<false><<<c->grid_stream, kBlock, 0, c->stream>>>(c->params, acc, c->lens, d);
	cudaError_t e = cudaGetLastError();
	if (e == cudaSuccess) e = cudaMemcpyAsync(out_host, d, n * sizeof(float), cudaMemcpyDeviceToHost, c->stream);
	if (e == cudaSuccess) e = sync_main(c);
	cudaFree(d); c->launches++;
	if (e != cudaSuccess) return fail(B2R_ERR_CUDA, cudaGetErrorString(e));
	return B2R_OK;
}

static int cover_ray_origins(b2r_ctx* c, const float* rays, uint32_t n) {
	float pts[6] = {FLT_MAX, FLT_MAX, FLT_MAX, -FLT_MAX, -FLT_MAX, -FLT_MAX};
	for (uint32_t i = 0; i < n; i++) for (int k = 0; k < 3; k++) { const float v = rays[6 * static_cast<size_t>(i) + k]; if (v == v && fabsf(v) <= FLT_MAX) { pts[k] = fminf(pts[k], v); pts[3 + k] = fmaxf(pts[3 + k], v); } }
	return pts[0] <= pts[3] ? ensure_origin_box(c, pts, 2) : B2R_OK;
}
static int trace_common(b2r_ctx* c, const float* rays, const float* tfar_in, uint32_t n, int shadow, float* tfar_out, int32_t* prim_out, uint8_t* occ_out) {
	if (!c || !rays) return fail(B2R_ERR_ARG, "null argument");
	if (!c->have_scene) return fail(B2R_ERR_STATE, "upload_scene first");
	if (n == 0) return B2R_OK;
	int rc = ensure_device(c); if (rc) return rc;
	if (c->use_bvh && (rc = cover_ray_origins(c, rays, n))) return rc;
	c->main_reads_scene = true;
	const size_t n6 = (static_cast<size_t>(n) * 6 * sizeof(float) + 255) & ~static_cast<size_t>(255), n4 = (static_cast<size_t>(n) * 4 + 255) & ~static_cast<size_t>(255), n1 = (static_cast<size_t>(n) + 255) & ~static_cast<size_t>(255);
	if ((rc = dev_reserve(&c->d_trace, &c->cap_trace, n6 + 3 * n4 + n1))) return rc;
	float* d_rays = reinterpret_cast<float*>(c->d_trace); float* d_tin = reinterpret_cast<float*>(c->d_trace + n6); float* d_tout = reinterpret_cast<float*>(c->d_trace + n6 + n4);
	int32_t* d_prim = reinterpret_cast<int32_t*>(c->d_trace + n6 + 2 * n4); uint8_t* d_occ = c->d_trace + n6 + 3 * n4;
	cudaError_t e = cudaMemcpyAsync(d_rays, rays, static_cast<size_t>(n) * 6 * sizeof(float), cudaMemcpyHostToDevice, c->stream);
	if (e == cudaSuccess && shadow) e = cudaMemcpyAsync(d_tin, tfar_in, static_cast<size_t>(n) * sizeof(float), cudaMemcpyHostToDevice, c->stream);
	if (e == cudaSuccess) {
		k_tap_trace<<<c->grid_stream, kBlock, 0, c->stream>>>(c->params.scene, d_rays, d_tin, n, c->use_bvh ? 1 : 0, shadow, d_tout, d_prim, d_occ);
		e = cudaGetLastError(); c->launches++;
	}
	if (e == cudaSuccess && !shadow) { e = cudaMemcpyAsync(tfar_out, d_tout, static_cast<size_t>(n) * sizeof(float), cudaMemcpyDeviceToHost, c->stream); if (e == cudaSuccess) e = cudaMemcpyAsync(prim_out, d_prim, static_cast<size_t>(n) * sizeof(int32_t), cudaMemcpyDeviceToHost, c->stream); }
	if (e == cudaSuccess && shadow) e = cudaMemcpyAsync(occ_out, d_occ, static_cast<size_t>(n), cudaMemcpyDeviceToHost, c->stream);
	if (e == cudaSuccess) e = sync_main(c);
	if (e != cudaSuccess) return fail(B2R_ERR_CUDA, cudaGetErrorString(e));
	return B2R_OK;
}
int b2r_trace_closest(b2r_ctx* c, const float* rays_host, uint32_t n, float* tfar_out, int32_t* prim_out) {
	if (!tfar_out || !prim_out) return fail(B2R_ERR_ARG, "null argument");
	return trace_common(c, rays_host, nullptr, n, 0, tfar_out, prim_out, nullptr);
}
int b2r_trace_shadow(b2r_ctx* c, const float* rays_host, const float* tfar_host, uint32_t n, uint8_t* occluded_out) {
	if (!tfar_host || !occluded_out) return fail(B2R_ERR_ARG, "null argument");
	return trace_common(c, rays_host, tfar_host, n, 1, nullptr, nullptr, occluded_out);
}
constexpr uint32_t kTapChunk = 1u << 16;
int b2r_trace_kernel(b2r_ctx* c, int kernel, const float* rays, const float* tfar, const int32_t* origin_prim, const uint8_t* tail,
                     uint32_t n, uint32_t acc, float* tfar_out, int32_t* prim_out, uint8_t* occluded_out) {
	if (!c) return fail(B2R_ERR_ARG, "null context");
	const bool closest = kernel == B2R_TAP_CLOSEST, shadow = kernel == B2R_TAP_SHADOW, packet = kernel == B2R_TAP_PACKET;
	if (!closest && !shadow && !packet) return fail(B2R_ERR_ARG, "unknown traversal kernel");
	if ((!packet && !rays) || (shadow ? (!tfar || !origin_prim || !occluded_out) : (!tfar_out || !prim_out))) return fail(B2R_ERR_ARG, "null argument");
	if (!c->have_scene) return fail(B2R_ERR_STATE, "upload_scene first");
	if (!c->use_bvh) return fail(B2R_ERR_STATE, "the traversal kernels run on BVH contexts only");
	if (packet && !c->have_camera) return fail(B2R_ERR_STATE, "set_camera first");
	if (packet && n != c->params.frame.npix) return fail(B2R_ERR_ARG, "packet kernel: n must be width * height");
	const uint32_t n_prims = c->params.scene.n_prims;
	if (shadow) for (uint32_t i = 0; i < n; i++) if (origin_prim[i] >= static_cast<int32_t>(n_prims)) return fail(B2R_ERR_ARG, "origin_prim out of range");
	if (n == 0) return B2R_OK;
	int rc = ensure_device(c); if (rc) return rc;
	if (!packet && (rc = cover_ray_origins(c, rays, n))) return rc;
	cudaStream_t st = c->stream;
	std::vector<uint32_t> leaf_node;
	if (shadow) { leaf_node.resize(n_prims); CU(cudaMemcpyAsync(leaf_node.data(), c->tables.leaf_node.p, n_prims * sizeof(uint32_t), cudaMemcpyDeviceToHost, st)); CU(sync_main(c)); }
	c->main_reads_scene = true;
	const uint32_t chunk = packet ? n : std::min(n, kTapChunk), cap = (chunk + 255u) & ~255u;
	size_t off = 0; auto take = [&](size_t bytes) { const size_t at = off; off += (bytes + 255u) & ~static_cast<size_t>(255u); return at; };
	const size_t o_a = take(cap * sizeof(float4)), o_b = take(cap * sizeof(float4)), o_t = take(3u * cap * sizeof(float)), o_h = take(cap * sizeof(float2)),
	             o_sa = take(cap * sizeof(float4)), o_sb = take(cap * sizeof(float4)), o_sl = take(3u * cap * sizeof(float)), o_ss = take(cap * sizeof(uint32_t)),
	             o_rad = take(3u * cap * sizeof(float)), o_slot = take(cap), o_act = take(cap / 256u * sizeof(uint16_t)), o_cnt = take(16u * sizeof(uint32_t)),
	             o_stats = take(ST_COUNT * sizeof(unsigned long long)), o_batch = take((1u + kMaxLanes) * sizeof(BatchDev));
	if ((rc = dev_reserve(&c->d_tap, &c->cap_tap, off))) return rc;
	uint8_t* base = c->d_tap;
	Params p = c->params;
	p.q.A[0] = p.q.A[1] = reinterpret_cast<float4*>(base + o_a); p.q.B[0] = p.q.B[1] = reinterpret_cast<float4*>(base + o_b); p.q.T[0] = p.q.T[1] = reinterpret_cast<float*>(base + o_t);
	p.q.H = reinterpret_cast<float2*>(base + o_h); p.q.SA = reinterpret_cast<float4*>(base + o_sa); p.q.SB = reinterpret_cast<float4*>(base + o_sb);
	p.q.SL = reinterpret_cast<float*>(base + o_sl); p.q.SS = reinterpret_cast<uint32_t*>(base + o_ss); p.q.cap = cap;
	p.rad = reinterpret_cast<float*>(base + o_rad);
	p.ex.slot[0] = p.ex.slot[1] = base + o_slot; p.ex.act[0] = p.ex.act[1] = reinterpret_cast<uint16_t*>(base + o_act);
	uint32_t* cnt = reinterpret_cast<uint32_t*>(base + o_cnt);
	p.cnt.paths = cnt; p.cnt.shadow = cnt + 4; p.cnt.work_a = cnt + 8; p.cnt.work_b = cnt + 12;
	p.cnt.stats = reinterpret_cast<unsigned long long*>(base + o_stats);
	BatchDev* batch = reinterpret_cast<BatchDev*>(base + o_batch); p.batch = batch;
	const KernelSet k = pick_kernels(c);
	std::vector<float2> h(chunk);
	if (packet) {
		BatchArgs a; a.n = 1u; a.acc[0] = acc; a.cam = c->params.frame.cam; a.lens = c->lens;
		k_set_batch<<<1, kMaxSlots, 0, st>>>(batch, a);
		CU(cudaMemsetAsync(cnt, 0, 16u * sizeof(uint32_t), st));
		k.packet<<<k.g_packet, kTravBlock, 0, st>>>(p, 0u);
		CU(cudaGetLastError()); c->launches += 2;
		CU(cudaMemcpyAsync(h.data(), p.q.H, n * sizeof(float2), cudaMemcpyDeviceToHost, st));
		CU(sync_main(c));
		for (uint32_t i = 0; i < n; i++) { tfar_out[i] = h[i].x; std::memcpy(&prim_out[i], &h[i].y, sizeof(int32_t)); }
		return B2R_OK;
	}
	p.frame.npix = cap; p.frame.npix_magic = magic_for(cap);
	std::vector<float4> ha(chunk), hb(chunk);
	std::vector<uint32_t> hs(chunk);
	std::vector<uint8_t> hslot(chunk);
	std::vector<float> hrad(chunk);
	if (shadow) { const std::vector<float> ones(3u * static_cast<size_t>(cap), 1.0f); CU(cudaMemcpyAsync(p.q.SL, ones.data(), ones.size() * sizeof(float), cudaMemcpyHostToDevice, st)); CU(sync_main(c)); }
	else {
		const std::vector<uint16_t> act(cap / 256u, static_cast<uint16_t>(8u));
		CU(cudaMemcpyAsync(p.ex.act[1], act.data(), act.size() * sizeof(uint16_t), cudaMemcpyHostToDevice, st)); CU(sync_main(c));
	}
	for (uint32_t first = 0; first < n; first += chunk) {
		const uint32_t m = std::min(chunk, n - first);
		for (uint32_t i = 0; i < m; i++) {
			const float* r = rays + 6 * static_cast<size_t>(first + i);
			float pid; const uint32_t pid_i = i; std::memcpy(&pid, &pid_i, sizeof pid);
			ha[i] = make_float4(r[0], r[1], r[2], r[3]);
			hb[i] = make_float4(r[4], r[5], shadow ? tfar[first + i] : 0.0f, pid);
			if (shadow) { const int32_t o = origin_prim[first + i]; hs[i] = o < 0 ? 0u : leaf_node[o]; }
			else hslot[i] = tail && tail[first + i] ? 255u : 0u;
		}
		uint32_t counts[16] = {0};
		if (shadow) counts[4] = m; else counts[1] = m;
		CU(cudaMemcpyAsync(cnt, counts, sizeof counts, cudaMemcpyHostToDevice, st));
		CU(cudaMemcpyAsync(shadow ? p.q.SA : p.q.A[1], ha.data(), m * sizeof(float4), cudaMemcpyHostToDevice, st));
		CU(cudaMemcpyAsync(shadow ? p.q.SB : p.q.B[1], hb.data(), m * sizeof(float4), cudaMemcpyHostToDevice, st));
		if (shadow) {
			CU(cudaMemcpyAsync(p.q.SS, hs.data(), m * sizeof(uint32_t), cudaMemcpyHostToDevice, st));
			CU(cudaMemsetAsync(p.rad, 0, 3u * static_cast<size_t>(cap) * sizeof(float), st));
			k.shadow<<<c->grid_shadow, kTravBlock, 0, st>>>(p, 0u);
			CU(cudaGetLastError()); c->launches++;
			CU(cudaMemcpyAsync(hrad.data(), p.rad, m * sizeof(float), cudaMemcpyDeviceToHost, st));
			CU(sync_main(c));
			for (uint32_t i = 0; i < m; i++) occluded_out[first + i] = hrad[i] == 0.0f ? 1u : 0u;
		} else {
			CU(cudaMemcpyAsync(p.ex.slot[1], hslot.data(), m, cudaMemcpyHostToDevice, st));
			k.closest<<<c->grid_closest, kTravBlock, 0, st>>>(p, 1u);
			CU(cudaGetLastError()); c->launches++;
			CU(cudaMemcpyAsync(h.data(), p.q.H, m * sizeof(float2), cudaMemcpyDeviceToHost, st));
			CU(sync_main(c));
			for (uint32_t i = 0; i < m; i++) { tfar_out[first + i] = h[i].x; std::memcpy(&prim_out[first + i], &h[i].y, sizeof(int32_t)); }
		}
	}
	return B2R_OK;
}
int b2r_read_link_tables(b2r_ctx* c, uint32_t* parent_out, uint32_t* leaf_node_out) {
	if (!c || !parent_out || !leaf_node_out) return fail(B2R_ERR_ARG, "null argument");
	if (!c->have_scene) return fail(B2R_ERR_STATE, "upload_scene first");
	if (!c->use_bvh) return fail(B2R_ERR_STATE, "a brute-force context has no traversal tree");
	int rc = ensure_device(c); if (rc) return rc;
	c->main_reads_scene = true;
	CU(cudaMemcpyAsync(parent_out, c->tables.parent.p, static_cast<size_t>(c->n_wide) * sizeof(uint32_t), cudaMemcpyDeviceToHost, c->stream));
	CU(cudaMemcpyAsync(leaf_node_out, c->tables.leaf_node.p, static_cast<size_t>(c->params.scene.n_prims) * sizeof(uint32_t), cudaMemcpyDeviceToHost, c->stream));
	CU(sync_main(c));
	return B2R_OK;
}
int b2r_get_origin_box(b2r_ctx* c, float out[6]) {
	if (!c || !out) return fail(B2R_ERR_ARG, "null argument");
	if (!c->obox_valid) return fail(B2R_ERR_STATE, "upload_scene first");
	for (int k = 0; k < 3; k++) { out[k] = c->obox.lo[k]; out[3 + k] = c->obox.hi[k]; }
	return B2R_OK;
}
int b2r_read_wide_nodes(b2r_ctx* c, void* out_host, uint32_t* n_wide_nodes, uint32_t* max_stack) {
	if (!c) return fail(B2R_ERR_ARG, "null context");
	if (!c->have_scene) return fail(B2R_ERR_STATE, "upload_scene first");
	if (n_wide_nodes) *n_wide_nodes = c->n_wide;
	if (max_stack) *max_stack = c->wide_host.max_stack;
	if (out_host && c->wide_refit) {
		int rc = ensure_device(c); if (rc) return rc;
		c->main_reads_scene = true;
		CU(cudaMemcpyAsync(out_host, c->tables.wide.p, static_cast<size_t>(c->n_wide) * sizeof(WideNode), cudaMemcpyDeviceToHost, c->stream));
		CU(sync_main(c));
	} else if (out_host) std::memcpy(out_host, c->wide_host.nodes.data(), c->wide_host.nodes.size() * sizeof(WideNode));
	return B2R_OK;
}

}
```

cpu-raytracing-experiments_b200/csrc/b2r_device.cuh:

```cuda
#pragma once
#include <cuda_runtime.h>
#include "b2r_shade.h"

namespace b2r {

constexpr int kBruteTile = 256;
constexpr int kBlock = 256;
constexpr int kTravBlock = 128;

__device__ __forceinline__ uint32_t lane_id() { return threadIdx.x & 31u; }

__device__ __forceinline__ void stat_add(unsigned long long* stats, int which, uint32_t v) {
	const uint32_t s = __reduce_add_sync(0xffffffffu, v);
	if (lane_id() == 0 && s) atomicAdd(stats + which, static_cast<unsigned long long>(s));
}

__device__ __forceinline__ uint32_t smem_addr(const void* p) {
	uint32_t a; asm volatile("mov.u32 %0, %1;" : "=r"(a) : "r"(static_cast<uint32_t>(__cvta_generic_to_shared(p))));
	return a;
}
__device__ __forceinline__ float4 lds_f4(uint32_t addr) {
	float4 v; asm volatile("ld.shared.v4.f32 {%0, %1, %2, %3}, [%4];" : "=f"(v.x), "=f"(v.y), "=f"(v.z), "=f"(v.w) : "r"(addr));
	return v;
}
// ... 572 lines not shown
			float4 na[4], nb[4];
#pragma unroll
			for (int k = 0; k < 4; k++) { na[k] = ldg4(nd + 2 * k); nb[k] = ldg4(nd + 2 * k + 1); }
			uint32_t key[4], link[4];
#pragma unroll
			for (int k = 0; k < 4; k++) {
				const float4 a = na[k], b = nb[k];
				const int32_t l = __float_as_int(b.z);
				key[k] = 0xffffffffu; link[k] = static_cast<uint32_t>(l);
				float tn[RPL]; bool h[RPL]; bool any = false; uint32_t tmin = 0xffffffffu;
#pragma unroll
				for (int r = 0; r < RPL; r++) {
					slab(a, b, ix[r], iy[r], iz[r], nx[r], ny[r], nz[r], ax[r], ay[r], az[r], best[r], &tn[r], &h[r]);
					any = any || h[r]; tmin = min(tmin, h[r] ? __float_as_uint(tn[r]) : 0xffffffffu);
				}
				if (COUNT && l != kEmptyLink) c_box += RPL;
				if (__ballot_sync(0xffffffffu, any) == 0u) continue;
				if (l < 0) {
#pragma unroll
					for (int r = 0; r < RPL; r++) if (h[r]) {
						float d; if (COUNT) c_sphere++;
						const int ro = LENS ? r : 0;
						if (sphere_hit_closest(a.x, a.y, a.z, a.w, ox[ro], oy[ro], oz[ro], dx[r], dy[r], dz[r], &d) && (d < best[r] || (d == best[r] && ~l < prim[r]))) { best[r] = d; prim[r] = ~l; }
					}
				} else key[k] = __reduce_min_sync(0xffffffffu, tmin);
			}
			float fb = best[0];
#pragma unroll
			for (int r = 1; r < RPL; r++) fb = fmaxf(fb, best[r]);
			const uint32_t far_best = __reduce_max_sync(0xffffffffu, __float_as_uint(fb));
			B2R_CSWAP(key[0], link[0], key[1], link[1]); B2R_CSWAP(key[2], link[2], key[3], link[3]);
			B2R_CSWAP(key[0], link[0], key[2], link[2]); B2R_CSWAP(key[1], link[1], key[3], link[3]);
			B2R_CSWAP(key[1], link[1], key[2], link[2]);
			if (key[3] <= far_best) { if (lane_id() == 0) stack[sp] = make_uint2(link[3], key[3]); sp++; }
			if (key[2] <= far_best) { if (lane_id() == 0) stack[sp] = make_uint2(link[2], key[2]); sp++; }
			if (key[1] <= far_best) { if (lane_id() == 0) stack[sp] = make_uint2(link[1], key[1]); sp++; }
			__syncwarp();
			if (key[0] <= far_best) { node = link[0]; continue; }
			bool found = false;
			while (sp > 0u) {
				const uint2 e = stack[--sp];
				if (e.y <= far_best) { node = e.x; found = true; break; }
			}
			if (!found) break;
		}
#pragma unroll
		for (int r = 0; r < RPL; r++) p.q.H[idx0 + 32u * r] = make_float2(best[r], __int_as_float(prim[r]));
	}
	if (blockIdx.x == 0 && threadIdx.x == 0) { p.cnt.paths[0] = n_in; atomicAdd(p.cnt.stats + ST_EXT, static_cast<unsigned long long>(n_in)); }
	if (COUNT) { stat_add(p.cnt.stats, ST_SPHERE, c_sphere); stat_add(p.cnt.stats, ST_BOX, c_box); }
}

template <bool COUNT, bool EXACT, uint32_t TNB>
__global__ void __launch_bounds__(kTravBlock) k_intersect_closest(const Params p, const uint32_t bounce) {
	const uint32_t n_in = p.cnt.paths[bounce];
	const int side = bounce & 1;
	uint32_t c_sphere = 0, c_box = 0;
	using Walk = TravClosestT<SmemStack>;
	lane_walks<Walk>(p.scene.wide, p.cnt.work_a + bounce, n_in,
		[&](Walk& t, uint32_t idx) {
			const float4 a = p.q.A[side][idx], b = p.q.B[side][idx];
			bool tail = false;
			if (EXACT && bounce > 0u) {
				const uint32_t pid_i = __float_as_uint(b.w), stream = (pid_i >> 26) * (p.frame.npix >> 8) + ((pid_i & kPixMask) >> 8);
				tail = static_cast<uint32_t>(p.ex.slot[side][idx]) >= (static_cast<uint32_t>(p.ex.act[side][stream]) & ~7u);
			}
			t.begin(Ray{a.x, a.y, a.z, a.w, b.x, b.y}, tail);
		},
		[&](Walk& t, const float4* row) { return t.template step_staged<COUNT, TNB>(row, p.scene.stack_tn_bits, &c_sphere, &c_box); },
		[&](const Walk& t, uint32_t idx) { p.q.H[idx] = make_float2(t.best, __int_as_float(t.prim)); });
	if (blockIdx.x == 0 && threadIdx.x == 0) atomicAdd(p.cnt.stats + ST_EXT, static_cast<unsigned long long>(n_in));
	if (COUNT) { stat_add(p.cnt.stats, ST_SPHERE, c_sphere); stat_add(p.cnt.stats, ST_BOX, c_box); }
}
template <bool EXACT, bool GGX = false, bool DIELECTRIC = false>
__global__ void __launch_bounds__(kBruteBlock, B2R_SHADE_MIN_BLOCKS) k_shade(const Params p, const uint32_t bounce) {
	constexpr int kQ = 2 * kBruteBlock;
	__shared__ uint32_t s_hit_i[kQ]; __shared__ float s_hit_t[kQ]; __shared__ int32_t s_hit_prim[kQ];
	__shared__ uint32_t s_cnt_a[kBruteWarps], s_cnt_b[kBruteWarps], s_cnt_c[kBruteWarps], s_base, s_sbase;
	const SceneDev& sc = p.scene;
	const uint32_t n_in = p.cnt.paths[bounce];
	const int side = bounce & 1;
	const bool mis = !(p.frame.flags & B2R_FLAG_NO_MIS);
	const bool last = bounce + 1 >= p.frame.max_bounces;
	uint32_t c_hits = 0, c_term = 0, c_drop = 0, c_events = 0, c_inline_shadow = 0;
	if (blockIdx.x * kBruteBlock >= n_in) return;
	uint32_t queued = 0, base = blockIdx.x * kBruteBlock;
	for (;;) {
		const bool more = base < n_in;
		if (more) {
			const uint32_t i = base + threadIdx.x;
			const bool live = i < n_in;
			float depth = FLT_MAX; int32_t prim = -1;
			if (live) { const float2 h = p.q.H[i]; depth = h.x; prim = __float_as_int(h.y); }
			const bool is_hit = live && prim >= 0;
#ifndef B2R_NO_SHADE_PREFETCH
			if (is_hit) {
				prefetch_l1(p.q.A[side] + i); prefetch_l1(p.q.B[side] + i); prefetch_l1(p.q.T[side] + i); prefetch_l1(p.q.T[side] + p.q.cap + i); prefetch_l1(p.q.T[side] + 2u * p.q.cap + i);
				prefetch_l1(sc.prims + prim); prefetch_l1(sc.prim_mat + prim); prefetch_l1(sc.leaf_node + prim);
			}
			if (base + gridDim.x * kBruteBlock + threadIdx.x < n_in) prefetch_l1(p.q.H + base + gridDim.x * kBruteBlock + threadIdx.x);
#endif
			if (live && !is_hit) {
				c_term++;
				if (sc.has_ambient) { const PathState sm = load_path(p.q, side, i); rad_add(p.rad, p.frame.npix, sm.pid, shade_sky(sc, sm), f3{0.0f, 0.0f, 0.0f}, true, false); c_events++; }
			}
			uint32_t n_hits;
			const uint32_t slot = queued + block_rank(is_hit, s_cnt_a, &n_hits);
			if (is_hit) { s_hit_i[slot] = i; s_hit_t[slot] = depth; s_hit_prim[slot] = prim; }
			queued += n_hits;
			base += gridDim.x * kBruteBlock;
			__syncthreads();
		}
		if (queued < static_cast<uint32_t>(kBruteBlock) && more) continue;
		if (queued == 0) break;
		const uint32_t take = min(queued, static_cast<uint32_t>(kBruteBlock));
		const uint32_t qi = queued - take + threadIdx.x;
		const bool shade = threadIdx.x < take;
		queued -= take;
		bool keep = false, want_shadow = false; ShadowRay sr; PathState s; uint32_t pid = 0, ex_slot = 0, ex_mat = 0, start = 0;
		if (shade) {
			const uint32_t hi = s_hit_i[qi]; const float depth = s_hit_t[qi]; const int32_t prim = s_hit_prim[qi];
			start = __ldg(sc.leaf_node + prim);
			s = load_path(p.q, side, hi); pid = s.pid;
			if (EXACT) ex_slot = bounce == 0u ? (pid & 255u) : static_cast<uint32_t>(p.ex.slot[side][hi]);
			const uint32_t acc = p.batch->acc[s.pid >> 26], seed = pixel_seed(s.pid & kPixMask, p.frame.max_bounces);
			const Surface sf = shade_surface<GGX, DIELECTRIC>(sc, s, depth, prim, p.mat_diel);
			if (EXACT) ex_mat = static_cast<uint32_t>(sf.mat);
			c_hits++;
			if (last) { rad_zero(p.rad, p.frame.npix, s.pid); c_drop++; }
			else {
				if (mis) want_shadow = shade_light_sample<GGX, DIELECTRIC>(sc, sf, s, prim, acc, seed, bounce, &sr);
				if (sf.emissive) {
					const f3 emit = shade_emission<DIELECTRIC>(sc, sf, s, depth, bounce, mis);
					if (want_shadow) {
						uint32_t cs = 0, cb = 0;
						const bool occluded = traverse_any<false>(sc.wide, Ray{sr.o.x, sr.o.y, sr.o.z, sr.d.x, sr.d.y, sr.d.z}, sr.tfar, &cs, &cb, sc.parent, 0u);
						rad_add(p.rad, p.frame.npix, s.pid, sr.L, emit, !occluded, true);
						want_shadow = false; c_inline_shadow++;
					} else rad_add(p.rad, p.frame.npix, s.pid, emit, f3{0.0f, 0.0f, 0.0f}, true, false);
					c_events++;
				}
				keep = shade_continue<GGX, DIELECTRIC>(sf, &s, acc, seed, bounce);
				if (!keep) c_term++;
			}
		}
		uint32_t n_shadow, n_keep, srank, rank;
		block_rank2(want_shadow, keep, s_cnt_b, s_cnt_c, &srank, &n_shadow, &rank, &n_keep);
		if (threadIdx.x == 0) {
			s_sbase = n_shadow ? atomicAdd(p.cnt.shadow + bounce, n_shadow) : 0u;
			s_base = n_keep ? atomicAdd(p.cnt.paths + bounce + 1, n_keep) : 0u;
		}
		__syncthreads();
		if (want_shadow) {
			const uint32_t d = s_sbase + srank;
			p.q.SA[d] = make_float4(sr.o.x, sr.o.y, sr.o.z, sr.d.x);
			p.q.SB[d] = make_float4(sr.d.y, sr.d.z, sr.tfar, __uint_as_float(pid));
			p.q.SL[d] = sr.L.x; p.q.SL[p.q.cap + d] = sr.L.y; p.q.SL[2u * p.q.cap + d] = sr.L.z;
			p.q.SS[d] = start;
		}
		if (keep) {
			store_path(p.q, side ^ 1, s_base + rank, s);
			if (EXACT) {
				const uint32_t e = (pid >> 26) * p.frame.npix + ((pid & kPixMask) & ~255u) + ex_slot;
				p.ex.key[e] = static_cast<uint8_t>(ex_mat + 1u); p.ex.next_idx[e] = s_base + rank;
			}
		}
	}
	stat_add(p.cnt.stats, ST_HITS, c_hits); stat_add(p.cnt.stats, ST_TERM, c_term);
	stat_add(p.cnt.stats, ST_DROPPED, c_drop); stat_add(p.cnt.stats, ST_EVENTS, c_events); stat_add(p.cnt.stats, ST_SHADOW, c_inline_shadow);
}
template <bool COUNT>
__global__ void __launch_bounds__(kTravBlock, 8) k_intersect_shadow(const Params p, const uint32_t bounce) {
	const uint32_t n_in = p.cnt.shadow[bounce];
	const uint32_t* __restrict__ parent = p.scene.parent;
	uint32_t c_sphere = 0, c_box = 0, c_events = 0, pid = 0;
	using Walk = TravAnyT<SmemStack>;
	lane_walks<Walk>(p.scene.wide, p.cnt.work_b + bounce, n_in,
		[&](Walk& t, uint32_t idx) {
			const float4 a = p.q.SA[idx], b = p.q.SB[idx];
			pid = __float_as_uint(b.w);
			t.begin(Ray{a.x, a.y, a.z, a.w, b.x, b.y}, b.z, p.q.SS[idx], parent);
		},
		[&](Walk& t, const float4* row) { return t.template step_staged<COUNT>(row, parent, &c_sphere, &c_box); },
		[&](const Walk& t, uint32_t idx) {
			if (t.occluded) return;
			const f3 L{p.q.SL[idx], p.q.SL[p.q.cap + idx], p.q.SL[2u * p.q.cap + idx]};
			rad_add(p.rad, p.frame.npix, pid, L, f3{0.0f, 0.0f, 0.0f}, true, false); c_events++;
		});
	if (blockIdx.x == 0 && threadIdx.x == 0) atomicAdd(p.cnt.stats + ST_SHADOW, static_cast<unsigned long long>(n_in));
	stat_add(p.cnt.stats, ST_EVENTS, c_events);
	if (COUNT) { stat_add(p.cnt.stats, ST_SPHERE, c_sphere); stat_add(p.cnt.stats, ST_BOX, c_box); }
}


__global__ void __launch_bounds__(kBlock) k_accumulate(const Params p) {
	__shared__ uint32_t s_order[kMaxSlots];
	__shared__ uint32_t s_first[kMaxSlots + 1];
	const uint32_t npix4 = p.frame.npix / 4u, n = 3u * npix4, slots = p.batch->n_slots, K = p.frame.buckets;
	if (threadIdx.x == 0) {
		uint32_t m = 0;
		const unsigned long long fold = p.batch->fold;
		for (uint32_t k = 0; k < K; k++) { s_first[k] = m; for (uint32_t s = 0; s < slots; s++) if (((fold >> s) & 1ull) && p.batch->acc[s] % K == k) s_order[m++] = s; }
		s_first[K] = m;
	}
	__syncthreads();
	const float4* __restrict__ rad = reinterpret_cast<const float4*>(p.rad); float4* __restrict__ acc = reinterpret_cast<float4*>(p.acc);
	const float4 zero = make_float4(0.0f, 0.0f, 0.0f, 0.0f);
	for (uint32_t i = blockIdx.x * blockDim.x + threadIdx.x; i < n; i += gridDim.x * blockDim.x) {
		const uint32_t c = i / npix4, t4 = i - c * npix4;
		for (uint32_t k = 0; k < K; k++) {
			const uint32_t b0 = s_first[k], b1 = s_first[k + 1];
			if (b0 == b1) continue;
			float4* dst = acc + (static_cast<size_t>(k) * 3u + c) * npix4 + t4;
			float4 sum = *dst;
			for (uint32_t j = b0; j < b1; j += 4u) {
				float4 v[4];
#pragma unroll
				for (uint32_t u = 0; u < 4u; u++) v[u] = (j + u < b1) ? rad[(static_cast<size_t>(s_order[j + u]) * 3u + c) * npix4 + t4] : zero;
#pragma unroll
				for (uint32_t u = 0; u < 4u; u++) if (j + u < b1) { sum.x += v[u].x; sum.y += v[u].y; sum.z += v[u].z; sum.w += v[u].w; }
			}
			*dst = sum;
		}
	}
}
struct BucketPtrs { const float* k[64]; };
__device__ __forceinline__ float median_buckets_at(const BucketPtrs& bp, uint32_t K, uint32_t off) {
	if (K == 5) return median_of_5(bp.k[0][off], bp.k[1][off], bp.k[2][off], bp.k[3][off], bp.k[4][off]);
	if (K == 3) return median_of_3(bp.k[0][off], bp.k[1][off], bp.k[2][off]);
	if (K == 1) return bp.k[0][off];
	if (K == 8) return median_of_8(bp.k[0][off], bp.k[1][off], bp.k[2][off], bp.k[3][off], bp.k[4][off], bp.k[5][off], bp.k[6][off], bp.k[7][off]);
	float v[64];
	for (uint32_t k = 0; k < K; k++) {
		float x = bp.k[k][off]; int j = static_cast<int>(k) - 1;
		while (j >= 0 && v[j] > x) { v[j + 1] = v[j]; j--; }
		v[j + 1] = x;
	}
	return (K & 1u) ? v[K / 2u] : (v[K / 2u - 1u] + v[K / 2u]) * 0.5f;
}
__global__ void __launch_bounds__(kBlock) k_resolve(const FrameDev frame, const __grid_constant__ BucketPtrs bp, float4* __restrict__ fb, const float scale, const int tonemap,
                                                    const uint32_t t_begin, const uint32_t t_end) {
	const uint32_t npix = frame.npix, K = frame.buckets;
	for (uint32_t t = t_begin + blockIdx.x * blockDim.x + threadIdx.x; t < t_end; t += gridDim.x * blockDim.x) {
		float r = scale * median_buckets_at(bp, K, t);
		float g = scale * median_buckets_at(bp, K, npix + t);
		float b = scale * median_buckets_at(bp, K, 2u * npix + t);
		if (tonemap) aces_tonemap(&r, &g, &b);
		int32_t x, y; pixel_xy(t, frame, &x, &y);
		fb[static_cast<size_t>(y) * frame.width + x] = make_float4(r, g, b, 1.0f);
	}
}

constexpr int kTeamMax = 16;
struct TeamSync {
	uint32_t ready[kTeamMax];
	uint32_t done[kTeamMax];
	uint32_t copied;
	uint32_t error;
};
struct TeamPeers { TeamSync* sync[kTeamMax]; };
enum TeamField { TEAM_READY = 0, TEAM_DONE = 1, TEAM_COPIED = 2 };
constexpr long long kTeamSpinLimit = 8000000000ll;
__device__ __forceinline__ uint32_t ld_acquire_sys(const uint32_t* p) { uint32_t v; asm volatile("ld.acquire.sys.global.u32 %0, [%1];" : "=r"(v) : "l"(p) : "memory"); return v; }
__device__ __forceinline__ void st_release_sys(uint32_t* p, uint32_t v) { asm volatile("st.release.sys.global.u32 [%0], %1;" ::"l"(p), "r"(v) : "memory"); }
__global__ void k_team_signal(const __grid_constant__ TeamPeers peers, const uint32_t n_ranks, const uint32_t my_rank, const int field, const uint32_t frame) {
	const uint32_t r = threadIdx.x;
	if (r >= n_ranks) return;
	__threadfence_system();
// ... 257 lines not shown
```

cpu-raytracing-experiments_b200/csrc/b2r_shade.h:

```cpp
#pragma once
#include <vector_types.h>
#include <vector_functions.h>
#include "b2r_math.h"
#include "b2r_host.h"

namespace b2r {

constexpr int kMaxSlots = 64;
constexpr uint32_t kPixMask = (1u << 26) - 1u;

B2R_HD int32_t as_int(float f) { return static_cast<int32_t>(bits(f)); }
B2R_HD float from_int(int32_t v) { return from_bits(static_cast<uint32_t>(v)); }
B2R_HD float4 ldg4(const float4* p) {
#if defined(__CUDA_ARCH__)
	return __ldg(p);
#else
	return *p;
#endif
}
B2R_HD uint32_t ldg_u32(const uint32_t* p) {
#if defined(__CUDA_ARCH__)
	return __ldg(p);
#else
	return *p;
#endif
}
B2R_HD float4 ld4(const float4* p) { return *p; }

enum Stat { ST_EXT = 0, ST_SHADOW, ST_HITS, ST_TERM, ST_DROPPED, ST_SPHERE, ST_BOX, ST_EVENTS, ST_COUNT };

struct SceneDev {
	const float4* prims;
	const int32_t* prim_mat;
	const float4* mat_albedo;
	const float4* mat_emission;
	const float4* mat_f0;
	const float4* light_sphere;
	const float4* light_emit;
	const WideNode* wide;
	const uint32_t* parent;
	const uint32_t* leaf_node;
	const float4* hdri;
	uint32_t n_prims, n_mat, n_lights;
	uint32_t stack_tn_bits;
	float light_sel_pdf;
	float ambient[3]; int32_t has_ambient;
	int32_t hdri_w, hdri_h; float hdri_fw, hdri_fh;
};
struct FrameDev {
	CameraParams cam;
	uint32_t width, height, h_tiles, npix;
	uint32_t max_bounces, buckets, flags;
	uint32_t h_tiles_magic, npix_magic;
	uint32_t finish_below, finish_first;
};
B2R_HD uint32_t div_by(uint32_t x, uint32_t d, uint32_t magic) {
#if defined(__CUDA_ARCH__)
	uint32_t q = __umulhi(x, magic);
#else
	uint32_t q = static_cast<uint32_t>((static_cast<uint64_t>(x) * magic) >> 32);
#endif
	if (x - q * d >= d) q++;
	return q;
}
B2R_HD uint32_t magic_for(uint32_t d) { return d <= 1u ? 0xffffffffu : static_cast<uint32_t>((1ull << 32) / d); }
struct BatchDev {
	uint32_t n_slots;
	uint32_t acc[kMaxSlots];
	CameraParams cam;
	LensParams lens;
	unsigned long long fold;
};
struct QueueDev {
	float4* A[2]; float4* B[2]; float* T[2];
	float2* H;
	float4* SA; float4* SB; float* SL;
	uint32_t* SS;
	uint32_t cap;
};
struct CountDev {
	uint32_t* paths;
	uint32_t* shadow;
	uint32_t* work_a;
	uint32_t* work_b;
	unsigned long long* stats;
};
struct ExactDev {
	uint8_t* slot[2];
	uint16_t* act[2];
	uint8_t* key;
	uint32_t* next_idx;
};
struct Params {
	SceneDev scene; FrameDev frame; QueueDev q; CountDev cnt; ExactDev ex;
	const BatchDev* batch;
	float* rad;
	float* acc;
	const float4* mat_diel;
};

B2R_HD void pixel_xy(uint32_t t, const FrameDev& fr, int32_t* x, int32_t* y) {
	const uint32_t tile = t >> 8, id = t & 255u;
	const uint32_t ty = div_by(tile, fr.h_tiles, fr.h_tiles_magic), tx = tile - ty * fr.h_tiles;
	*x = static_cast<int32_t>(tx * 16u + (id & 15u));
	*y = static_cast<int32_t>(ty * 16u + (id >> 4));
}

struct PathState { float ox, oy, oz, dx, dy, dz, tr, tg, tb, pdf; uint32_t pid; };

template <bool LENS = false>
B2R_HD PathState primary_path(const FrameDev& fr, const CameraParams& cam, uint32_t acc, uint32_t slot, uint32_t t, const LensParams& lens = LensParams{0.0f, 0.0f}) {
	Pcg rng{hash_2d(acc, pixel_seed(t, fr.max_bounces))};
	const float s0 = rng.next_unit(), s1 = rng.next_unit();
	int32_t x, y; pixel_xy(t, fr, &x, &y);
	PathState s;
	if constexpr (LENS) {
		Pcg lr{hash_2d(acc, pixel_seed(t, fr.max_bounces) + 2u * fr.max_bounces)};
		const float u0 = lr.next_unit(), u1 = lr.next_unit();
		f3 o, d; camera_lens_ray(cam, x, y, s0, s1, lens, u0, u1, &o, &d);
		s.ox = o.x; s.oy = o.y; s.oz = o.z; s.dx = d.x; s.dy = d.y; s.dz = d.z;
	} else {
		const f3 d = camera_dir(cam, x, y, s0, s1);
		s.ox = cam.px; s.oy = cam.py; s.oz = cam.pz; s.dx = d.x; s.dy = d.y; s.dz = d.z;
	}
	s.tr = s.tg = s.tb = 1.0f; s.pdf = 0.0f; s.pid = (slot << 26) | t;
	return s;
}


struct Surface {
	f3 P; TangentQuat T; float n_dot_v; f3 albedo; bool emissive; int32_t mat; float r2; f3 v_local; float alpha;
	bool inside; float4 diel; f3 P_in;
};
struct ShadowRay { f3 o, d; float tfar; f3 L; };

B2R_HD bool dielectric_scatter(f3 v, float r, float u0, f3* dir, float* F) {
	const float c = sel_min(sel_max(v.z, 0.0f), 1.0f);
	const float s2 = r * r * (1.0f - c * c);
	if (s2 >= 1.0f) { *F = 1.0f; *dir = f3{-v.x, -v.y, c}; return true; }
	const float ct = sqrtf(1.0f - s2);
	const float rs = (r * c - ct) / (r * c + ct), rp = (r * ct - c) / (r * ct + c);
	*F = (rs * rs + rp * rp) * 0.5f;
	const bool refl = u0 < *F;
	*dir = refl ? f3{-v.x, -v.y, c} : f3{-r * v.x, -r * v.y, -ct};
	return refl;
}

template <bool GGX = false, bool DIELECTRIC = false>
B2R_HD Surface shade_surface(const SceneDev& sc, const PathState& s, float depth, int32_t prim, const float4* mat_diel = nullptr) {
	const float4 sp = ld4(sc.prims + prim);
	const f3 D{s.dx, s.dy, s.dz};
	const f3 hp{s.ox + D.x * depth, s.oy + D.y * depth, s.oz + D.z * depth};
	f3 N = unit3(f3{hp.x - sp.x, hp.y - sp.y, hp.z - sp.z});
	const bool flip = dot3(N, D) >= 0.0f;
	if (flip) N = f3{-N.x, -N.y, -N.z};
	Surface sf;
	sf.T = tangent_frame(N);
	const f3 vl = frame_to_local(sf.T, f3{-D.x, -D.y, -D.z});
	sf.n_dot_v = vl.z;
	sf.P = f3{hp.x + N.x * 1e-4f, hp.y + N.y * 1e-4f, hp.z + N.z * 1e-4f};
	sf.mat = sc.prim_mat[prim];
	const float4 al = ld4(sc.mat_albedo + sf.mat);
	sf.albedo = f3{al.x, al.y, al.z}; sf.emissive = al.w != 0.0f; sf.r2 = sp.w;
	if (GGX) {
		const float4 fr = ld4(sc.mat_f0 + sf.mat);
		float alpha = fr.w; alpha *= alpha;
		sf.albedo = f3{fr.x, fr.y, fr.z}; sf.alpha = alpha + (1.0f - alpha) * 0.0f; sf.v_local = vl;
	}
	if (DIELECTRIC) {
		sf.diel = ld4(mat_diel + sf.mat); sf.inside = flip; sf.v_local = vl;
		sf.P_in = f3{hp.x - N.x * 1e-4f, hp.y - N.y * 1e-4f, hp.z - N.z * 1e-4f};
	}
	return sf;
}
template <bool DIELECTRIC> B2R_HD bool is_dielectric(const Surface& sf) { return DIELECTRIC && sf.diel.w != 0.0f; }
template <bool GGX = false, bool DIELECTRIC = false>
B2R_HD bool shade_light_sample(const SceneDev& sc, const Surface& sf, const PathState& s, int32_t hit_prim,
                                                   uint32_t acc, uint32_t seed, uint32_t bounce, ShadowRay* out) {
	if (is_dielectric<DIELECTRIC>(sf)) return false;
	if (sc.n_lights == 0u) return false;
	Pcg rng{hash_2d(acc, seed + bounce * 2u)};
	const float u0 = rng.next_unit(), u1 = rng.next_unit();
	const uint32_t pick = rng.next_below(sc.n_lights);
	const float4 ls = ld4(sc.light_sphere + pick), le = ld4(sc.light_emit + pick);
	if (as_int(le.w) == hit_prim) return false;
	f3 wc{ls.x - sf.P.x, ls.y - sf.P.y, ls.z - sf.P.z};
	const float d2 = dot3(wc, wc);
	if (d2 <= ls.w) return false;
	const float dist = sqrtf(d2);
	wc = scale3(wc, 1.0f / dist);
	const float sin2 = ls.w / d2;
	const float n_dot_w = (2.0f * sf.T.w) * (wc.z * sf.T.w + wc.x * sf.T.y - sf.T.x * wc.y) - wc.z;
	if (n_dot_w < 0.0f && sin2 < n_dot_w * n_dot_w) return false;
	float ldist, lpdf;
	const f3 L = sample_sphere_cone(wc, sin2, dist, ls.w, u0, u1, &ldist, &lpdf);
	const f3 ll = frame_to_local(sf.T, L);
	if (ll.z < 0.0f) return false;
	f3 rad{le.x * s.tr, le.y * s.tg, le.z * s.tb};
	if (GGX) { const f3 e = ggx_eval(sf.albedo, sf.alpha, ll, sf.v_local); rad = f3{rad.x * e.x, rad.y * e.y, rad.z * e.z}; }
	else {
		const float f = B2R_INV_PI * sel_max(0.0f, ll.z);
		rad = f3{rad.x * (sf.albedo.x * f), rad.y * (sf.albedo.y * f), rad.z * (sf.albedo.z * f)};
	}
	lpdf *= sc.light_sel_pdf;
	const float bpdf = GGX ? 0.0f : B2R_INV_PI * sel_max(0.0f, ll.z);
	const float w = power_heuristic_over_f(lpdf, bpdf);
	rad = scale3(rad, w);
	if (sel_max(sel_max(rad.x, rad.y), rad.z) <= 0.0f) return false;
	out->o = sf.P; out->d = L; out->tfar = ldist; out->L = rad;
	return true;
}
template <bool DIELECTRIC = false>
B2R_HD f3 shade_emission(const SceneDev& sc, const Surface& sf, const PathState& s, float depth, uint32_t bounce, bool mis) {
	const float4 em = ld4(sc.mat_emission + sf.mat);
	if (!mis) return f3{s.tr * em.x, s.tg * em.y, s.tb * em.z};
	if (bounce == 0) return f3{em.x, em.y, em.z};
	if (DIELECTRIC && s.pdf < 0.0f) return f3{s.tr * em.x, s.tg * em.y, s.tb * em.z};
	const float d2 = depth * (depth + sf.n_dot_v * (2.0f * sqrtf(sf.r2))) + sf.r2;
	const float w = power_heuristic(s.pdf, sc.light_sel_pdf * sphere_light_pdf(sf.r2, d2));
	return f3{(s.tr * w) * em.x, (s.tg * w) * em.y, (s.tb * w) * em.z};
}
template <bool GGX = false, bool DIELECTRIC = false>
B2R_HD bool shade_continue(const Surface& sf, PathState* s, uint32_t acc, uint32_t seed, uint32_t bounce) {
	Pcg rng{hash_2d(acc, seed + bounce * 2u + 1u)};
	const float u0 = rng.next_unit(), u1 = rng.next_unit();
	f3 dl, est = sf.albedo, o = sf.P;
	const bool delta = is_dielectric<DIELECTRIC>(sf);
	if (delta) {
		float F;
		if (dielectric_scatter(sf.v_local, sf.inside ? sf.diel.w : 1.0f / sf.diel.w, u0, &dl, &F)) est = f3{1.0f, 1.0f, 1.0f};
		else { est = f3{sf.diel.x, sf.diel.y, sf.diel.z}; o = sf.P_in; }
	}
	else if (GGX) ggx_sample(sf.albedo, sf.alpha, sf.v_local, u0, u1, &dl, &est);
	else dl = cosine_hemisphere(u0, u1);
	f3 thr{s->tr * est.x, s->tg * est.y, s->tb * est.z};
	const float q = 1.0f - sel_max(thr.x, sel_max(thr.y, thr.z));
	if (rng.next_unit() < q) return false;
	thr = scale3(thr, 1.0f / sel_max(FLT_EPSILON, 1.0f - q));
	const f3 dw = frame_to_world(sf.T, dl);
	s->ox = o.x; s->oy = o.y; s->oz = o.z; s->dx = dw.x; s->dy = dw.y; s->dz = dw.z;
	s->tr = thr.x; s->tg = thr.y; s->tb = thr.z;
	s->pdf = delta ? -1.0f : GGX ? 0.0f : B2R_INV_PI * sel_max(0.0f, dw.z);
	return true;
}
B2R_HD f3 shade_sky(const SceneDev& sc, const PathState& s) {
	const float u = sc.hdri_fw * (0.5f + B2R_INV_TWO_PI * atan2_poly(s.dz, s.dx));
	const float v = sc.hdri_fh * (0.5f - B2R_INV_PI * asin_poly(s.dy));
	const float4 tx = ldg4(sc.hdri + (static_cast<int32_t>(v) * sc.hdri_w + static_cast<int32_t>(u)));
	return f3{s.tr * (tx.x * sc.ambient[0]), s.tr * (tx.y * sc.ambient[1]), s.tr * (tx.z * sc.ambient[2])};
}
B2R_HD void rad_add(float* rad, uint32_t npix, uint32_t pid, f3 a, f3 b, bool has_a = true, bool has_b = true) {
	const uint32_t slot = pid >> 26, t = pid & kPixMask;
	float* r = rad + static_cast<size_t>(slot) * 3u * npix + t;
#if defined(__CUDA_ARCH__)
	if (has_a) { atomicAdd(r, a.x); atomicAdd(r + npix, a.y); atomicAdd(r + 2u * npix, a.z); }
	if (has_b) { atomicAdd(r, b.x); atomicAdd(r + npix, b.y); atomicAdd(r + 2u * npix, b.z); }
#else
	if (has_a) { r[0] += a.x; r[npix] += a.y; r[2u * npix] += a.z; }
	if (has_b) { r[0] += b.x; r[npix] += b.y; r[2u * npix] += b.z; }
#endif
}
B2R_HD void rad_zero(float* rad, uint32_t npix, uint32_t pid) {
	const uint32_t slot = pid >> 26, t = pid & kPixMask;
	float* r = rad + static_cast<size_t>(slot) * 3u * npix + t;
	r[0] = 0.0f; r[npix] = 0.0f; r[2u * npix] = 0.0f;
}

struct Ray { float ox, oy, oz, dx, dy, dz; };

constexpr float kSlabWiden = 1.0000008f;
constexpr float kSlabReach = 18446744073709551616.0f;
constexpr float kSlabRange = 8.50705917302346159e37f;
B2R_HD void slab_setup(float ox, float oy, float oz, float dx, float dy, float dz, float* ix, float* iy, float* iz, float* nx, float* ny, float* nz,
                       float* ax, float* ay, float* az) {
	const float sx = 1.0f / dx, sy = 1.0f / dy, sz = 1.0f / dz;
	const float reach = ((fabsf(ox) + fabsf(oy)) + fabsf(oz)) + kSlabReach;
	const float nan = from_bits(0x7fc00000u);
	*ix = sx; *iy = sy; *iz = sz;
	*nx = fabsf(sx) * reach <= kSlabRange ? -(ox * sx) : nan;
	*ny = fabsf(sy) * reach <= kSlabRange ? -(oy * sy) : nan;
	*nz = fabsf(sz) * reach <= kSlabRange ? -(oz * sz) : nan;
	*ax = fabsf(sx); *ay = fabsf(sy); *az = fabsf(sz);
}
B2R_HD void slab(const float4 a, const float4 b, float ix, float iy, float iz, float nx, float ny, float nz, float ax, float ay, float az,
                 float limit, float* tnear, bool* hit) {
	const float cx = fma_rn(a.x, ix, nx), cy = fma_rn(a.y, iy, ny), cz = fma_rn(a.z, iz, nz);
	const float t0 = fmaxf(fmaxf(fmaxf(fma_rn(-b.x, ax, cx), fma_rn(-b.y, ay, cy)), fma_rn(-b.w, az, cz)), 0.0f);
	const float t1 = fminf(fminf(fminf(fma_rn(b.x, ax, cx), fma_rn(b.y, ay, cy)), fma_rn(b.w, az, cz)), limit);
	*tnear = t0; *hit = t0 <= t1 * kSlabWiden;
}
#define B2R_CSWAP(ka, la, kb, lb) { const bool sw = kb < ka; const uint32_t tk = sw ? kb : ka, tl = sw ? lb : la; kb = sw ? ka : kb; lb = sw ? la : lb; ka = tk; la = tl; }

constexpr uint32_t kMaxWideNodes = 1u << 22;
// ... 3 lines not shown
	B2R_HD void push(uint32_t v) { e[sp++] = v; }
	B2R_HD uint32_t pop() { return e[--sp]; }
	B2R_HD bool empty() const { return sp == 0; }
	B2R_HD void room() {}
	B2R_HD bool refill() { return false; }
};
B2R_HD uint32_t pack_entry(uint32_t node, uint32_t tnear_bits, uint32_t tn_bits) { return (node << tn_bits) | (tnear_bits >> (31u - tn_bits)); }
B2R_HD float entry_tnear(uint32_t e, uint32_t tn_bits) { return from_bits((e & ((1u << tn_bits) - 1u)) << (31u - tn_bits)); }
B2R_HD uint32_t entry_node(uint32_t e, uint32_t tn_bits) { return e >> tn_bits; }

struct TravBase {
	float ox, oy, oz, dx, dy, dz;
	float ix, iy, iz, nx, ny, nz;
	float ax, ay, az;
	uint32_t node;
	B2R_HD void arm(const Ray& r) {
		ox = r.ox; oy = r.oy; oz = r.oz; dx = r.dx; dy = r.dy; dz = r.dz;
		slab_setup(r.ox, r.oy, r.oz, r.dx, r.dy, r.dz, &ix, &iy, &iz, &nx, &ny, &nz, &ax, &ay, &az);
		node = 0u;
	}
};
template <bool STAGED> B2R_HD float4 node_f4(const float4* n, int i) { return STAGED ? n[i] : ldg4(n + i); }
B2R_HD int first_bit(uint32_t m) {
#if defined(__CUDA_ARCH__)
	return __ffs(static_cast<int>(m)) - 1;
#else
	return __builtin_ctz(m);
#endif
}

template <class Stack>
struct TravClosestT : TravBase {
	float best; int32_t prim;
	bool tail = false;
	Stack stack;
	B2R_HD void begin(const Ray& r, bool scalar_tail = false) { arm(r); best = FLT_MAX; prim = -1; tail = scalar_tail; stack.reset(); }
	template <bool COUNT, bool STAGED, uint32_t TNB = 0u>
	B2R_HD bool visit(const float4* n, uint32_t tn_bits_rt, uint32_t* c_sphere, uint32_t* c_box) {
		const uint32_t tn_bits = TNB ? TNB : tn_bits_rt;
		uint32_t key[4], link[4]; uint32_t leaves = 0u;
#pragma unroll
		for (int k = 0; k < 4; k++) {
			const float4 a = node_f4<STAGED>(n, 2 * k), b = node_f4<STAGED>(n, 2 * k + 1);
			const int32_t l = as_int(b.z);
			float tn; bool h; slab(a, b, ix, iy, iz, nx, ny, nz, ax, ay, az, best, &tn, &h);
			if (COUNT && l != kEmptyLink) (*c_box)++;
			key[k] = (h && l >= 0) ? bits(tn) : 0xffffffffu; link[k] = static_cast<uint32_t>(l);
			leaves |= (h && l < 0) ? (1u << k) : 0u;
		}
		while (leaves) {
			const int k = first_bit(leaves);
			leaves &= leaves - 1u;
			const float4 sp = node_f4<STAGED>(n, 2 * k); const int32_t id = ~as_int(node_f4<STAGED>(n, 2 * k + 1).z);
			float d; if (COUNT) (*c_sphere)++;
			const bool cand = tail ? sphere_hit_closest_scalar(sp.x, sp.y, sp.z, sp.w, ox, oy, oz, dx, dy, dz, &d) : sphere_hit_closest(sp.x, sp.y, sp.z, sp.w, ox, oy, oz, dx, dy, dz, &d);
			if (cand) {
				if (d < best || (d == best && id < prim)) { best = d; prim = id; }
			}
		}
		B2R_CSWAP(key[0], link[0], key[1], link[1]); B2R_CSWAP(key[2], link[2], key[3], link[3]);
		B2R_CSWAP(key[0], link[0], key[2], link[2]); B2R_CSWAP(key[1], link[1], key[3], link[3]);
		B2R_CSWAP(key[1], link[1], key[2], link[2]);
		stack.room();
		if (from_bits(key[3]) <= best) stack.push(pack_entry(link[3], key[3], tn_bits));
		if (from_bits(key[2]) <= best) stack.push(pack_entry(link[2], key[2], tn_bits));
		if (from_bits(key[1]) <= best) stack.push(pack_entry(link[1], key[1], tn_bits));
		if (from_bits(key[0]) <= best) { node = link[0]; return true; }
		for (;;) {
			while (!stack.empty()) {
				const uint32_t e = stack.pop();
				if (entry_tnear(e, tn_bits) <= best) { node = entry_node(e, tn_bits); return true; }
			}
			if (!stack.refill()) return false;
		}
	}
	template <bool COUNT>
	B2R_HD bool step(const WideNode* __restrict__ wide, uint32_t tn_bits, uint32_t* c_sphere, uint32_t* c_box) { return visit<COUNT, false>(reinterpret_cast<const float4*>(wide + node), tn_bits, c_sphere, c_box); }
	template <bool COUNT, uint32_t TNB = 0u>
	B2R_HD bool step_staged(const float4* n, uint32_t tn_bits, uint32_t* c_sphere, uint32_t* c_box) { return visit<COUNT, true, TNB>(n, tn_bits, c_sphere, c_box); }
};
constexpr uint32_t kNoNode = 0xffffffffu;
template <class Stack>
struct TravAnyT : TravBase {
	float tfar; bool occluded;
	uint32_t root, up, skip;
	Stack stack;
	B2R_HD void begin(const Ray& r, float limit, uint32_t start, const uint32_t* __restrict__ parent) {
		arm(r); tfar = limit; occluded = false; stack.reset();
		node = root = start; up = start != 0u ? ldg_u32(parent + start) : 0u; skip = kNoNode;
	}
	template <bool COUNT, bool STAGED>
	B2R_HD bool visit(const float4* n, const uint32_t* __restrict__ parent, uint32_t* c_sphere, uint32_t* c_box) {
		uint32_t next = kNoNode, leaves = 0u; float next_tn = FLT_MAX;
		stack.room();
#pragma unroll
		for (int k = 0; k < 4; k++) {
			const float4 a = node_f4<STAGED>(n, 2 * k), b = node_f4<STAGED>(n, 2 * k + 1);
			const int32_t l = as_int(b.z);
			float tn; bool h; slab(a, b, ix, iy, iz, nx, ny, nz, ax, ay, az, tfar, &tn, &h);
			if (COUNT && l != kEmptyLink) (*c_box)++;
			if (h && l >= 0 && static_cast<uint32_t>(l) != skip) {
				const bool nearer = tn < next_tn;
				const uint32_t later = nearer ? next : static_cast<uint32_t>(l);
				if (later != kNoNode) stack.push(later);
				if (nearer) { next = static_cast<uint32_t>(l); next_tn = tn; }
			}
			leaves |= (h && l < 0) ? (1u << k) : 0u;
		}
		while (leaves) {
			const int k = first_bit(leaves);
			leaves &= leaves - 1u;
			const float4 sp = node_f4<STAGED>(n, 2 * k);
			if (COUNT) (*c_sphere)++;
			if (sphere_hit_any(sp.x, sp.y, sp.z, sp.w, ox, oy, oz, dx, dy, dz, tfar)) { occluded = true; return false; }
		}
		if (next == kNoNode && (!stack.empty() || stack.refill())) next = stack.pop();
		if (next == kNoNode && root != 0u) { skip = root; root = up; next = up; up = ldg_u32(parent + up); }
		node = next;
		return next != kNoNode;
	}
	template <bool COUNT>
	B2R_HD bool step(const WideNode* __restrict__ wide, const uint32_t* __restrict__ parent, uint32_t* c_sphere, uint32_t* c_box) { return visit<COUNT, false>(reinterpret_cast<const float4*>(wide + node), parent, c_sphere, c_box); }
	template <bool COUNT>
	B2R_HD bool step_staged(const float4* n, const uint32_t* __restrict__ parent, uint32_t* c_sphere, uint32_t* c_box) { return visit<COUNT, true>(n, parent, c_sphere, c_box); }
};
using TravClosest = TravClosestT<ArrayStack>;
using TravAny = TravAnyT<ArrayStack>;
template <bool COUNT>
B2R_HD void traverse_closest(const WideNode* __restrict__ wide, uint32_t tn_bits, const Ray& r, float* best_out, int32_t* prim_out, uint32_t* c_sphere, uint32_t* c_box) {
	TravClosest t; t.begin(r);
	while (t.template step<COUNT>(wide, tn_bits, c_sphere, c_box)) {}
	*best_out = t.best; *prim_out = t.prim;
}
template <bool COUNT>
B2R_HD bool traverse_any(const WideNode* __restrict__ wide, const Ray& r, float tfar, uint32_t* c_sphere, uint32_t* c_box, const uint32_t* __restrict__ parent = nullptr, uint32_t start = 0u) {
	TravAny t; t.begin(r, tfar, start, parent);
	while (t.template step<COUNT>(wide, parent, c_sphere, c_box)) {}
	return t.occluded;
}

constexpr float kHitNoise = 1.5e-6f;
constexpr float kBoxPad = 4.0e-7f;
B2R_HD float leaf_half_extent(const float4 s , const OriginBox& ob) {
	const float ex = sel_max(fabsf(s.x - ob.lo[0]), fabsf(ob.hi[0] - s.x)), ey = sel_max(fabsf(s.y - ob.lo[1]), fabsf(ob.hi[1] - s.y)), ez = sel_max(fabsf(s.z - ob.lo[2]), fabsf(ob.hi[2] - s.z));
	const float far2 = (ex * ex + ey * ey + ez * ez) * 1.0001f;
	const float h = sqrtf(s.w + kHitNoise * far2);
	return h + (sel_max(fabsf(s.x), sel_max(fabsf(s.y), fabsf(s.z))) + h + 1.0f) * kBoxPad;
}
B2R_HD void refit_child_box(const float4* __restrict__ child , float4* a_out, float4* b_out, int32_t link) {
	float lx = FLT_MAX, ly = FLT_MAX, lz = FLT_MAX, hx = -FLT_MAX, hy = -FLT_MAX, hz = -FLT_MAX;
	for (int j = 0; j < 4; j++) {
		const float4 ca = child[2 * j], cb = child[2 * j + 1];
		if (static_cast<int32_t>(bits(cb.z)) == kEmptyLink) continue;
		lx = sel_min(lx, ca.x - cb.x); ly = sel_min(ly, ca.y - cb.y); lz = sel_min(lz, ca.z - cb.w);
		hx = sel_max(hx, ca.x + cb.x); hy = sel_max(hy, ca.y + cb.y); hz = sel_max(hz, ca.z + cb.w);
	}
	const float cx = 0.5f * (lx + hx), cy = 0.5f * (ly + hy), cz = 0.5f * (lz + hz);
	float ex = sel_max(hx - cx, cx - lx), ey = sel_max(hy - cy, cy - ly), ez = sel_max(hz - cz, cz - lz);
	ex += (fabsf(cx) + ex + 1.0f) * kBoxPad; ey += (fabsf(cy) + ey + 1.0f) * kBoxPad; ez += (fabsf(cz) + ez + 1.0f) * kBoxPad;
	*a_out = make_float4(cx, cy, cz, 0.0f); *b_out = make_float4(ex, ey, from_bits(static_cast<uint32_t>(link)), ez);
}
B2R_HD void refit_slot(float4* __restrict__ wide , const float4* __restrict__ prims, const uint32_t* __restrict__ remap, const OriginBox& ob, uint32_t node, int k) {
	float4* slot = wide + static_cast<size_t>(node) * 8 + 2 * k;
	const int32_t link = static_cast<int32_t>(bits(slot[1].z));
	if (link == kEmptyLink) return;
	if (link < 0) {
		const uint32_t now = remap ? remap[~link] : static_cast<uint32_t>(~link);
		const float4 s = prims[now]; const float h = leaf_half_extent(s, ob);
		slot[0] = s; slot[1] = make_float4(h, h, from_bits(~now), h);
		return;
	}
	float4 a, b; refit_child_box(wide + static_cast<size_t>(link) * 8, &a, &b, link);
	slot[0] = a; slot[1] = b;
}
B2R_HD uint32_t morton_spread10(uint32_t v) { v &= 1023u; v = (v | (v << 16)) & 0x030000ffu; v = (v | (v << 8)) & 0x0300f00fu; v = (v | (v << 4)) & 0x030c30c3u; v = (v | (v << 2)) & 0x09249249u; return v; }
B2R_HD uint32_t morton_key(float cx, float cy, float cz, const float lo[3], const float scale[3]) {
	const float fx = (cx - lo[0]) * scale[0], fy = (cy - lo[1]) * scale[1], fz = (cz - lo[2]) * scale[2];
	const uint32_t qx = static_cast<uint32_t>(sel_min(sel_max(fx, 0.0f), 1023.0f)), qy = static_cast<uint32_t>(sel_min(sel_max(fy, 0.0f), 1023.0f)), qz = static_cast<uint32_t>(sel_min(sel_max(fz, 0.0f), 1023.0f));
#if defined(B2R_MORTON_ORDER)
	return (morton_spread10(qx) << 2) | (morton_spread10(qy) << 1) | morton_spread10(qz);
#else
	uint32_t x0 = qx, x1 = qy, x2 = qz;
	for (uint32_t q = 512u; q > 1u; q >>= 1) {
		const uint32_t m = q - 1u; uint32_t t;
		if (x0 & q) x0 ^= m;
		if (x1 & q) x0 ^= m; else { t = (x0 ^ x1) & m; x0 ^= t; x1 ^= t; }
		if (x2 & q) x0 ^= m; else { t = (x0 ^ x2) & m; x0 ^= t; x2 ^= t; }
	}
	x1 ^= x0; x2 ^= x1;
	uint32_t t = 0u;
	for (uint32_t q = 512u; q > 1u; q >>= 1) if (x2 & q) t ^= q - 1u;
	x0 ^= t; x1 ^= t; x2 ^= t;
	return (morton_spread10(x0) << 2) | (morton_spread10(x1) << 1) | morton_spread10(x2);
#endif
}
struct SweepItem { float lo0, lo1, lo2; uint32_t pos; float hi0, hi1, hi2; uint32_t flag; };
B2R_HD SweepItem sweep_join(const SweepItem& a, const SweepItem& b) {
	if (b.flag) return b;
	SweepItem r;
	r.lo0 = sel_min(a.lo0, b.lo0); r.lo1 = sel_min(a.lo1, b.lo1); r.lo2 = sel_min(a.lo2, b.lo2);
	r.hi0 = sel_max(a.hi0, b.hi0); r.hi1 = sel_max(a.hi1, b.hi1); r.hi2 = sel_max(a.hi2, b.hi2);
	r.pos = a.pos; r.flag = a.flag;
	return r;
}
B2R_HD float sweep_area(const SweepItem& s) { const float ex = s.hi0 - s.lo0, ey = s.hi1 - s.lo1, ez = s.hi2 - s.lo2; return ex * ey + ey * ez + ez * ex; }
B2R_HD void sweep_sphere_box(const float4 s, SweepItem* it) {
	const float r = sqrtf(s.w);
	it->lo0 = s.x - r; it->lo1 = s.y - r; it->lo2 = s.z - r; it->hi0 = s.x + r; it->hi1 = s.y + r; it->hi2 = s.z + r; it->pos = 0u; it->flag = 0u;
}
B2R_HD unsigned long long sweep_key(float area_l, uint32_t n_l, float area_r, uint32_t n_r, uint32_t pos) {
	const float cost = area_l * static_cast<float>(n_l) + area_r * static_cast<float>(n_r);
	return (static_cast<unsigned long long>(bits(cost)) << 32) | pos;
}
struct SweepKids { uint32_t a[4], b[4], n; };
B2R_HD uint32_t sweep_open(SweepKids& K, const unsigned long long* cut_of, const float* area_of) {
	if (K.n >= 4u) return 0u;
	int pick = -1; float best = -1.0f;
	for (uint32_t k = 0; k < K.n; k++) if (K.b[k] - K.a[k] >= 2u) { const float ar = area_of[K.a[k]]; if (ar > best) { best = ar; pick = static_cast<int>(k); } }
	if (pick < 0) return 0u;
	const uint32_t pos = static_cast<uint32_t>(cut_of[K.a[pick]] & 0xffffffffull);
	K.a[K.n] = pos; K.b[K.n] = K.b[pick]; K.b[pick] = pos; K.n++;
// ... 31 lines not shown
```

include/b2r.h:

```cpp
#ifndef B2R_H_
#define B2R_H_

#include <stddef.h>
#include <stdint.h>

#ifdef __cplusplus
extern "C" {
#endif

#define B2R_ABI_VERSION 1

typedef struct b2r_sphere {
	float position[3];
	float radius_sq;
	int32_t material_ID;
	int32_t _pad[3];
} b2r_sphere;

typedef struct b2r_material {
	float albedo[3], F0[3], F80[3], emission[3], transmission[3];
	float roughness, IOR_minus_one;
	float _pad[7];
} b2r_material;

// ... 35 lines not shown
	B2R_OK = 0,
	B2R_ERR_ARG = -1,
	B2R_ERR_CUDA = -2,
	B2R_ERR_STATE = -3,
	B2R_ERR_NO_LIGHTS = -4,
	B2R_ERR_BVH = -5,
	B2R_ERR_NOT_READY = 1,
};

typedef struct b2r_ctx b2r_ctx;


int b2r_bvh_build(const b2r_sphere* geometry, uint32_t n, b2r_bvh_node* nodes_out, b2r_sphere* prims_out,
                  uint32_t* prim_ids_out, uint32_t* n_nodes_out);
int b2r_bvh_build_ex(const b2r_sphere* geometry, uint32_t n, uint32_t log_cluster_size, float cost_ratio, b2r_bvh_node* nodes_out,
                     b2r_sphere* prims_out, uint32_t* prim_ids_out, uint32_t* n_nodes_out);
int b2r_find_lights(const b2r_sphere* geometry, uint32_t n, const b2r_material* materials, uint32_t n_mat,
                    int32_t* out, uint32_t* n_out);
int b2r_camera_lookat(const float eye[3], const float dir[3], uint32_t width, uint32_t height, float focal_length_mm,
                      float exposure, float out11[11]);

int b2r_camera_ray(const float pos[3], const float orient_wxyz[4], float half_width, float half_height, float z,
                   int32_t x, int32_t y, const float samples[2], float origin_out[3], float dir_out[3]);

int  b2r_create(b2r_ctx** out, const b2r_config* cfg);
void b2r_destroy(b2r_ctx* ctx);
int  b2r_resize(b2r_ctx* ctx, uint32_t width, uint32_t height);
int  b2r_reset(b2r_ctx* ctx);
int  b2r_set_stream(b2r_ctx* ctx, void* cuda_stream);
int  b2r_sync(b2r_ctx* ctx);

int  b2r_upload_scene(b2r_ctx* ctx, const b2r_sphere* prims_bvh_order, const b2r_bvh_node* nodes, uint32_t n_prims,
                      uint32_t n_nodes, const b2r_material* materials, uint32_t n_mat, const int32_t* light_geom_idx,
                      uint32_t n_lights, const b2r_sphere* geometry, uint32_t n_geom, const float ambient[3],
                      const float* hdri_rgba, int32_t hdri_w, int32_t hdri_h);
int  b2r_refit_scene(b2r_ctx* ctx, const b2r_sphere* prims_bvh_order, uint32_t n_prims, const b2r_material* materials, uint32_t n_mat,
                     const int32_t* light_geom_idx, uint32_t n_lights, const b2r_sphere* geometry, uint32_t n_geom, float* quality_out);
int  b2r_set_camera(b2r_ctx* ctx, const float pos[3], const float orient_wxyz[4], float half_width, float half_height,
                    float z, float exposure);
int  b2r_set_lens(b2r_ctx* ctx, float lens_radius, float focus_distance);

int  b2r_accumulate(b2r_ctx* ctx, uint32_t n_samples);
int  b2r_resolve(b2r_ctx* ctx, float* rgba_out_host, int tonemap);
int  b2r_resolve_async(b2r_ctx* ctx, float* rgba_out_host, int tonemap);
int  b2r_frame_wait(b2r_ctx* ctx);
int  b2r_resolve_device(b2r_ctx* ctx, int tonemap);
int  b2r_resolve_from(b2r_ctx* ctx, const void* dev_buckets, float* rgba_out_host, int tonemap);

int  b2r_host_register(void* ptr, size_t bytes);
int  b2r_host_unregister(void* ptr);

int  b2r_get_accumulations(b2r_ctx* ctx, uint32_t* out);
int  b2r_set_accumulations(b2r_ctx* ctx, uint32_t acc);
int  b2r_read_buckets(b2r_ctx* ctx, float* out_host);
int  b2r_write_buckets(b2r_ctx* ctx, const float* in_host);
int  b2r_save_checkpoint(b2r_ctx* ctx, const char* path);
int  b2r_load_checkpoint(b2r_ctx* ctx, const char* path);
int  b2r_device_buckets(b2r_ctx* ctx, void** dev_ptr, size_t* bytes);
int  b2r_device_framebuffer(b2r_ctx* ctx, void** dev_ptr, size_t* bytes);
int  b2r_ipc_export_buckets(b2r_ctx* ctx, unsigned char handle_out[64]);
int  b2r_ipc_open_peers(b2r_ctx* ctx, const unsigned char* peer_handles, uint32_t n_peers, uint32_t my_rank);
int  b2r_ipc_close(b2r_ctx* ctx);
int  b2r_resolve_peers(b2r_ctx* ctx, float* rgba_out_host, int tonemap);
int  b2r_team_export(b2r_ctx* ctx, unsigned char handles_out[192]);
int  b2r_team_open(b2r_ctx* ctx, const unsigned char* all_handles , uint32_t n_ranks, uint32_t my_rank);
int  b2r_team_resolve(b2r_ctx* ctx, float* rgba_out_host, int tonemap, int async);
int  b2r_team_error(b2r_ctx* ctx, uint32_t* error_out);
int  b2r_team_close(b2r_ctx* ctx);
int  b2r_read_counters(b2r_ctx* ctx, uint64_t out[10]);
int  b2r_reset_counters(b2r_ctx* ctx);
int  b2r_read_bounce_counts(b2r_ctx* ctx, uint32_t* paths_out, uint32_t* shadow_out, uint32_t n);
int  b2r_read_kernel_times(b2r_ctx* ctx, double ms_out[8], uint64_t launches_out[8], int reset);
int  b2r_set_flags(b2r_ctx* ctx, uint32_t flags);

int  b2r_generate_rays(b2r_ctx* ctx, uint32_t acc, float* out_host);
int  b2r_trace_closest(b2r_ctx* ctx, const float* rays_host, uint32_t n, float* tfar_out, int32_t* prim_out);
int  b2r_trace_shadow(b2r_ctx* ctx, const float* rays_host, const float* tfar_host, uint32_t n, uint8_t* occluded_out);
enum { B2R_TAP_CLOSEST = 0, B2R_TAP_SHADOW = 1, B2R_TAP_PACKET = 2 };
int  b2r_trace_kernel(b2r_ctx* ctx, int kernel, const float* rays, const float* tfar, const int32_t* origin_prim, const uint8_t* tail,
                      uint32_t n, uint32_t acc, float* tfar_out, int32_t* prim_out, uint8_t* occluded_out);
int  b2r_read_wide_nodes(b2r_ctx* ctx, void* out_host, uint32_t* n_wide_nodes, uint32_t* max_stack);
int  b2r_read_link_tables(b2r_ctx* ctx, uint32_t* parent_out, uint32_t* leaf_node_out);
int  b2r_get_origin_box(b2r_ctx* ctx, float lo_hi_out[6]);

int  b2r_write_hdr(const char* path, const float* rgba, uint32_t width, uint32_t height);

int  b2r_read_hdr(const char* path, float* rgba_out, int32_t* width_out, int32_t* height_out);

const char* b2r_last_error(void);
int  b2r_abi_version(void);

#ifdef __cplusplus
}
#endif
#endif
```

Measured before the change: 5862.

## Add shadow-ray occluder hint cache to skip traversal for likely-occluded rays

Adds a device hash table, keyed by hit primitive and light pick, that remembers the last sphere found to occlude a shadow ray. During shading the cached occluder is tested first, and if it blocks the ray the shadow ray is never queued, which skips a BVH any-hit traversal. The shadow kernel writes occluders back into the table, which needs a per-ray key buffer and racy relaxed loads and stores. It costs extra memory (a table with 4M entries), extra global traffic, and a possible change in thread scheduling, and it is on by default except in exact mode.

```diff
diff --git a/__graft_entry__.py b/__graft_entry__.py
--- a/__graft_entry__.py
+++ b/__graft_entry__.py
@@ -31,10 +31,11 @@
     src = os.path.join(ROOT, "tests", "hostcheck", "hostcheck.cpp")
     out = os.path.join(ROOT, "tests", "hostcheck", "libhostcheck.so")
     cam = os.path.join(ROOT, "tests", "hostcheck", "mirror_camera.cpp")
-    deps = [src, cam] + [os.path.join(CSRC, f) for f in ("b2r_host.cpp", "b2r_shade.h", "b2r_math.h", "b2r_host.h")] + [os.path.join(PKG, "host", f) for f in ("Camera.hpp", "Core.hpp")]
+    hints = os.path.join(ROOT, "tests", "hostcheck", "shadow_hints.cpp")
+    deps = [src, cam, hints] + [os.path.join(CSRC, f) for f in ("b2r_host.cpp", "b2r_shade.h", "b2r_math.h", "b2r_host.h")] + [os.path.join(PKG, "host", f) for f in ("Camera.hpp", "Core.hpp")]
     if force or _newer(out, deps):
         subprocess.check_call(["g++", "-std=c++17", "-O2", "-ffp-contract=off", "-mavx2", "-mfma", "-fPIC", "-shared",
-                               "-I/usr/local/cuda/include", "-I", CSRC, "-I", os.path.join(PKG, "host"), src, cam, os.path.join(CSRC, "b2r_host.cpp"), "-o", out])
+                               "-I/usr/local/cuda/include", "-I", CSRC, "-I", os.path.join(PKG, "host"), src, cam, hints, os.path.join(CSRC, "b2r_host.cpp"), "-o", out])
     return out
 
 
diff --git a/cpu-raytracing-experiments_b200/b2r.py b/cpu-raytracing-experiments_b200/b2r.py
--- a/cpu-raytracing-experiments_b200/b2r.py
+++ b/cpu-raytracing-experiments_b200/b2r.py
@@ -19,13 +19,13 @@
 TAP_CLOSEST, TAP_SHADOW, TAP_PACKET = 0, 1, 2
 OK, ERR_ARG, ERR_CUDA, ERR_STATE, ERR_NO_LIGHTS, ERR_BVH, NOT_READY = 0, -1, -2, -3, -4, -5, 1
 KERNEL_KINDS = ["generate", "bounce_brute", "intersect_closest", "shade", "intersect_shadow", "accumulate", "resolve"]
-COUNTER_NAMES = ["extension_rays", "shadow_rays", "shaded_hits", "terminated", "dropped", "sphere_tests", "box_tests", "launches", "radiance_events", "reserved"]
+COUNTER_NAMES = ["extension_rays", "shadow_rays", "shaded_hits", "terminated", "dropped", "sphere_tests", "box_tests", "launches", "radiance_events", "shadow_hinted"]
 
 ABI_SYMBOLS = [
     "b2r_bvh_build", "b2r_bvh_build_ex", "b2r_find_lights", "b2r_camera_lookat", "b2r_camera_ray", "b2r_create", "b2r_destroy", "b2r_resize", "b2r_reset", "b2r_set_stream",
     "b2r_sync", "b2r_upload_scene", "b2r_refit_scene", "b2r_set_camera", "b2r_set_lens", "b2r_accumulate", "b2r_resolve", "b2r_resolve_async", "b2r_resolve_device", "b2r_frame_wait", "b2r_resolve_from", "b2r_ipc_export_buckets", "b2r_ipc_open_peers", "b2r_ipc_close", "b2r_resolve_peers", "b2r_team_export", "b2r_team_open", "b2r_team_resolve", "b2r_team_error", "b2r_team_close", "b2r_host_register", "b2r_host_unregister", "b2r_get_accumulations", "b2r_set_accumulations",
     "b2r_read_buckets", "b2r_write_buckets", "b2r_save_checkpoint", "b2r_load_checkpoint", "b2r_device_buckets", "b2r_device_framebuffer", "b2r_read_counters", "b2r_reset_counters", "b2r_read_bounce_counts",
-    "b2r_read_kernel_times", "b2r_set_flags", "b2r_generate_rays", "b2r_trace_closest", "b2r_trace_shadow", "b2r_trace_kernel", "b2r_read_wide_nodes", "b2r_read_link_tables", "b2r_get_origin_box",
+    "b2r_read_kernel_times", "b2r_set_flags", "b2r_generate_rays", "b2r_trace_closest", "b2r_trace_shadow", "b2r_trace_kernel", "b2r_read_wide_nodes", "b2r_read_link_tables", "b2r_get_origin_box", "b2r_fill_shadow_hints",
     "b2r_write_hdr", "b2r_read_hdr", "b2r_last_error", "b2r_abi_version",
 ]
 
@@ -61,7 +61,7 @@
             "b2r_host_register": [vp, C.c_size_t], "b2r_host_unregister": [vp], "b2r_get_accumulations": [vp, vp], "b2r_set_accumulations": [vp, u32], "b2r_read_buckets": [vp, vp], "b2r_write_buckets": [vp, vp],
             "b2r_device_buckets": [vp, vp, vp], "b2r_device_framebuffer": [vp, vp, vp], "b2r_read_counters": [vp, vp], "b2r_reset_counters": [vp], "b2r_read_bounce_counts": [vp, vp, vp, u32],
             "b2r_read_kernel_times": [vp, vp, vp, C.c_int], "b2r_set_flags": [vp, u32], "b2r_generate_rays": [vp, u32, vp],
-            "b2r_save_checkpoint": [vp, C.c_char_p], "b2r_load_checkpoint": [vp, C.c_char_p], "b2r_write_hdr": [C.c_char_p, vp, u32, u32], "b2r_read_hdr": [C.c_char_p, vp, vp, vp], "b2r_trace_closest": [vp, vp, u32, vp, vp], "b2r_trace_shadow": [vp, vp, vp, u32, vp], "b2r_trace_kernel": [vp, C.c_int, vp, vp, vp, vp, u32, u32, vp, vp, vp], "b2r_read_wide_nodes": [vp, vp, vp, vp], "b2r_read_link_tables": [vp, vp, vp], "b2r_get_origin_box": [vp, vp],
+            "b2r_save_checkpoint": [vp, C.c_char_p], "b2r_load_checkpoint": [vp, C.c_char_p], "b2r_write_hdr": [C.c_char_p, vp, u32, u32], "b2r_read_hdr": [C.c_char_p, vp, vp, vp], "b2r_trace_closest": [vp, vp, u32, vp, vp], "b2r_trace_shadow": [vp, vp, vp, u32, vp], "b2r_trace_kernel": [vp, C.c_int, vp, vp, vp, vp, u32, u32, vp, vp, vp], "b2r_read_wide_nodes": [vp, vp, vp, vp], "b2r_read_link_tables": [vp, vp, vp], "b2r_get_origin_box": [vp, vp], "b2r_fill_shadow_hints": [vp, vp, u32],
         }
         for name, args in sig.items():
             fn = getattr(L, name); fn.argtypes = args; fn.restype = C.c_int
@@ -329,6 +329,9 @@
         _check(lib().b2r_read_wide_nodes(self._h, _ptr(out), C.byref(n), C.byref(ms)))
         return out, ms.value
 
+    def fill_shadow_hints(self, values):
+        v = np.ascontiguousarray(values, np.uint32); _check(lib().b2r_fill_shadow_hints(self._h, _ptr(v), len(v)))
+
     def origin_box(self):
         out = np.zeros(6, np.float32); _check(lib().b2r_get_origin_box(self._h, _ptr(out))); return out
 
diff --git a/cpu-raytracing-experiments_b200/csrc/b2r.cu b/cpu-raytracing-experiments_b200/csrc/b2r.cu
--- a/cpu-raytracing-experiments_b200/csrc/b2r.cu
+++ b/cpu-raytracing-experiments_b200/csrc/b2r.cu
@@ -22,6 +22,7 @@
 enum KernelKind { KK_GENERATE = 0, KK_BRUTE, KK_CLOSEST, KK_SHADE, KK_SHADOW, KK_ACCUMULATE, KK_RESOLVE, KK_COUNT };
 
 constexpr uint32_t kMaxLanes = 4;
+constexpr uint32_t kShadowHintMask = (1u << 22) - 1u;
 struct BatchArgs {
 	uint32_t n; uint32_t acc[kMaxSlots]; unsigned long long fold = ~0ull; CameraParams cam; LensParams lens{0.0f, 0.0f};
 	uint32_t lanes = 0, lane_slots = 0, n_lane[kMaxLanes] = {0, 0, 0, 0};
@@ -111,6 +112,7 @@
 	float *d_T[2] = {nullptr, nullptr}, *d_SL = nullptr, *d_rad = nullptr, *d_acc = nullptr;
 	uint8_t *d_ex_slot[2] = {nullptr, nullptr}, *d_ex_key = nullptr; uint16_t* d_ex_act[2] = {nullptr, nullptr}; uint32_t* d_ex_next = nullptr;
 	float2* d_H = nullptr; uint32_t* d_SS = nullptr;
+	uint32_t *d_hint = nullptr, *d_SK = nullptr; bool shadow_hints = true;
 	uint32_t* d_counts = nullptr; size_t counts_bytes = 0;
 	unsigned long long* d_stats = nullptr;
 	BatchDev* d_batch = nullptr;
@@ -188,6 +190,10 @@
 	if ((rc = dev_alloc(&c->d_SB, cap))) return rc;
 	if ((rc = dev_alloc(&c->d_SL, 3 * cap))) return rc;
 	if ((rc = dev_alloc(&c->d_SS, cap))) return rc;
+	if (c->shadow_hints) {
+		if ((rc = dev_alloc(&c->d_SK, cap))) return rc;
+		if (!c->d_hint) { if ((rc = dev_alloc(&c->d_hint, static_cast<size_t>(kShadowHintMask) + 1u))) return rc; CU(cudaMemset(c->d_hint, 0xff, (static_cast<size_t>(kShadowHintMask) + 1u) * sizeof(uint32_t))); }
+	}
 	if ((rc = dev_alloc(&c->d_rad, 3 * cap))) return rc;
 	if ((rc = dev_alloc(&c->d_acc, static_cast<size_t>(K) * 3 * npix))) return rc;
 	if ((rc = dev_alloc(&c->d_fb, static_cast<size_t>(npix)))) return rc;
@@ -215,6 +221,7 @@
 	}
 	for (int s = 0; s < 2; s++) { p.q.A[s] = c->d_A[s]; p.q.B[s] = c->d_B[s]; p.q.T[s] = c->d_T[s]; }
 	p.q.H = c->d_H; p.q.SA = c->d_SA; p.q.SB = c->d_SB; p.q.SL = c->d_SL; p.q.SS = c->d_SS; p.q.cap = static_cast<uint32_t>(cap);
+	p.shadow_hint = c->d_hint; p.shadow_hint_mask = kShadowHintMask; p.SK = c->d_SK;
 	p.cnt.paths = c->d_counts; p.cnt.shadow = c->d_counts + (mb + 1); p.cnt.work_a = c->d_counts + 2 * (mb + 1); p.cnt.work_b = c->d_counts + 3 * (mb + 1);
 	p.cnt.stats = c->d_stats;
 	p.batch = c->d_batch; p.rad = c->d_rad; p.acc = c->d_acc;
@@ -258,6 +265,7 @@
 	}
 	c->packet_primary = std::getenv("B2R_NO_PACKET") == nullptr;
 	c->lanes_max = std::getenv("B2R_NO_TWIN") ? 1u : 2u;
+	c->shadow_hints = std::getenv("B2R_NO_SHADOW_HINT") == nullptr;
 	if (const char* e = std::getenv("B2R_SIDES")) { c->sides = std::atoi(e) == 1 ? 1u : 2u; }
 	if (const char* e = std::getenv("B2R_LANES")) { const int v = std::atoi(e); if (v == 1 || v == 2 || v == 4) { c->lanes_max = static_cast<uint32_t>(v); c->lanes_forced = true; } }
 	if (const char* e = std::getenv("B2R_LANE_GRID")) { c->lane_grid_frac = static_cast<float>(std::atof(e)); if (!(c->lane_grid_frac > 0.0f && c->lane_grid_frac <= 1.0f)) c->lane_grid_frac = 1.0f; }
@@ -323,6 +331,7 @@
 	const KernelSet k = pick_kernels(c);
 	const uint32_t mb = c->cfg.max_bounces;
 	Params p = p_in;
+	if (exact) p.shadow_hint = nullptr;
 	int rc;
 	auto run = [&](int kind, BounceKernel fn, int grid, int block, uint32_t b) { return launch(c, kind, profile, [&] { fn<<<grid, block, 0, st>>>(p, b); }); };
 	if (!c->use_bvh) {
@@ -358,6 +367,7 @@
 	const size_t npix = p.frame.npix, off = static_cast<size_t>(side * cap_slots + rel) * npix, cap = static_cast<size_t>(mine) * npix;
 	for (int s = 0; s < 2; s++) { p.q.A[s] += off; p.q.B[s] += off; p.q.T[s] += 3 * off; }
 	p.q.H += off; p.q.SA += off; p.q.SB += off; p.q.SL += 3 * off; p.q.SS += off; p.q.cap = static_cast<uint32_t>(cap);
+	if (p.SK) p.SK += off;
 	const uint32_t block = (c->cfg.max_bounces + 1u) * 4u, blk = side * kMaxLanes + which;
 	p.cnt.paths += blk * block; p.cnt.shadow += blk * block; p.cnt.work_a += blk * block; p.cnt.work_b += blk * block;
 	p.batch = c->d_batch + side * (1u + kMaxLanes) + 1u + which;
@@ -745,7 +755,7 @@
 	dev_free(&c->d_cost); dev_free(&c->d_remap); dev_free(&c->d_trace); dev_free(&c->d_tap); dev_free(&c->d_cost_base); dev_free(&c->d_sort_tmp); dev_free(&c->d_sweep);
 	for (int k = 0; k < 2; k++) { dev_free(&c->d_mkey[k]); dev_free(&c->d_midx[k]); }
 	for (int s = 0; s < 2; s++) { dev_free(&c->d_A[s]); dev_free(&c->d_B[s]); dev_free(&c->d_T[s]); }
-	dev_free(&c->d_H); dev_free(&c->d_SA); dev_free(&c->d_SB); dev_free(&c->d_SL); dev_free(&c->d_SS); dev_free(&c->d_rad); dev_free(&c->d_acc); dev_free(&c->d_fb);
+	dev_free(&c->d_H); dev_free(&c->d_SA); dev_free(&c->d_SB); dev_free(&c->d_SL); dev_free(&c->d_SS); dev_free(&c->d_SK); dev_free(&c->d_hint); dev_free(&c->d_rad); dev_free(&c->d_acc); dev_free(&c->d_fb);
 	for (int s = 0; s < 2; s++) { dev_free(&c->d_ex_slot[s]); dev_free(&c->d_ex_act[s]); }
 	dev_free(&c->d_ex_key); dev_free(&c->d_ex_next);
 	dev_free(&c->d_counts); dev_free(&c->d_stats); dev_free(&c->d_batch);
@@ -1403,7 +1413,7 @@
 	CU(cudaMemcpyAsync(h, c->d_stats, sizeof h, cudaMemcpyDeviceToHost, c->stream));
 	CU(sync_main(c));
 	out[0] = h[ST_EXT]; out[1] = h[ST_SHADOW]; out[2] = h[ST_HITS]; out[3] = h[ST_TERM]; out[4] = h[ST_DROPPED]; out[5] = h[ST_SPHERE]; out[6] = h[ST_BOX];
-	out[7] = c->launches; out[8] = h[ST_EVENTS]; out[9] = 0;
+	out[7] = c->launches; out[8] = h[ST_EVENTS]; out[9] = h[ST_HINTED];
 	return collect_timings(c);
 }
 int b2r_read_bounce_counts(b2r_ctx* c, uint32_t* paths_out, uint32_t* shadow_out, uint32_t n) {
@@ -1520,6 +1530,7 @@
 	p.q.H = reinterpret_cast<float2*>(base + o_h); p.q.SA = reinterpret_cast<float4*>(base + o_sa); p.q.SB = reinterpret_cast<float4*>(base + o_sb);
 	p.q.SL = reinterpret_cast<float*>(base + o_sl); p.q.SS = reinterpret_cast<uint32_t*>(base + o_ss); p.q.cap = cap;
 	p.rad = reinterpret_cast<float*>(base + o_rad);
+	p.shadow_hint = nullptr;
 	p.ex.slot[0] = p.ex.slot[1] = base + o_slot; p.ex.act[0] = p.ex.act[1] = reinterpret_cast<uint16_t*>(base + o_act);
 	uint32_t* cnt = reinterpret_cast<uint32_t*>(base + o_cnt);
 	p.cnt.paths = cnt; p.cnt.shadow = cnt + 4; p.cnt.work_a = cnt + 8; p.cnt.work_b = cnt + 12;
@@ -1593,6 +1604,17 @@
 	CU(sync_main(c));
 	return B2R_OK;
 }
+int b2r_fill_shadow_hints(b2r_ctx* c, const uint32_t* values, uint32_t n) {
+	if (!c || !values || n == 0) return fail(B2R_ERR_ARG, "null argument");
+	if (!c->d_hint) return fail(B2R_ERR_STATE, "shadow hints are off (B2R_NO_SHADOW_HINT)");
+	int rc = ensure_device(c); if (rc) return rc;
+	const size_t m = static_cast<size_t>(kShadowHintMask) + 1u;
+	std::vector<uint32_t> h(m);
+	for (size_t i = 0; i < m; i++) h[i] = values[i % n];
+	CU(cudaMemcpyAsync(c->d_hint, h.data(), m * sizeof(uint32_t), cudaMemcpyHostToDevice, c->stream));
+	CU(sync_main(c));
+	return B2R_OK;
+}
 int b2r_get_origin_box(b2r_ctx* c, float out[6]) {
 	if (!c || !out) return fail(B2R_ERR_ARG, "null argument");
 	if (!c->obox_valid) return fail(B2R_ERR_STATE, "upload_scene first");
diff --git a/cpu-raytracing-experiments_b200/csrc/b2r_device.cuh b/cpu-raytracing-experiments_b200/csrc/b2r_device.cuh
--- a/cpu-raytracing-experiments_b200/csrc/b2r_device.cuh
+++ b/cpu-raytracing-experiments_b200/csrc/b2r_device.cuh
@@ -678,7 +678,7 @@
 	const int side = bounce & 1;
 	const bool mis = !(p.frame.flags & B2R_FLAG_NO_MIS);
 	const bool last = bounce + 1 >= p.frame.max_bounces;
-	uint32_t c_hits = 0, c_term = 0, c_drop = 0, c_events = 0, c_inline_shadow = 0;
+	uint32_t c_hits = 0, c_term = 0, c_drop = 0, c_events = 0, c_inline_shadow = 0, c_hinted = 0;
 	if (blockIdx.x * kBruteBlock >= n_in) return;
 	uint32_t queued = 0, base = blockIdx.x * kBruteBlock;
 	for (;;) {
@@ -713,7 +713,7 @@
 		const uint32_t qi = queued - take + threadIdx.x;
 		const bool shade = threadIdx.x < take;
 		queued -= take;
-		bool keep = false, want_shadow = false; ShadowRay sr; PathState s; uint32_t pid = 0, ex_slot = 0, ex_mat = 0, start = 0;
+		bool keep = false, want_shadow = false; ShadowRay sr; PathState s; uint32_t pid = 0, ex_slot = 0, ex_mat = 0, start = 0, hkey = 0;
 		if (shade) {
 			const uint32_t hi = s_hit_i[qi]; const float depth = s_hit_t[qi]; const int32_t prim = s_hit_prim[qi];
 			start = __ldg(sc.leaf_node + prim);
@@ -736,6 +736,7 @@
 					} else rad_add(p.rad, p.frame.npix, s.pid, emit, f3{0.0f, 0.0f, 0.0f}, true, false);
 					c_events++;
 				}
+				if (!EXACT && want_shadow && p.shadow_hint && shadow_hint_resolves(sc, p.shadow_hint, p.shadow_hint_mask, prim, sr, &hkey)) { want_shadow = false; c_hinted++; }
 				keep = shade_continue<GGX, DIELECTRIC>(sf, &s, acc, seed, bounce);
 				if (!keep) c_term++;
 			}
@@ -753,6 +754,7 @@
 			p.q.SB[d] = make_float4(sr.d.y, sr.d.z, sr.tfar, __uint_as_float(pid));
 			p.q.SL[d] = sr.L.x; p.q.SL[p.q.cap + d] = sr.L.y; p.q.SL[2u * p.q.cap + d] = sr.L.z;
 			p.q.SS[d] = start;
+			if (!EXACT && p.shadow_hint) p.SK[d] = hkey;
 		}
 		if (keep) {
 			store_path(p.q, side ^ 1, s_base + rank, s);
@@ -763,7 +765,8 @@
 		}
 	}
 	stat_add(p.cnt.stats, ST_HITS, c_hits); stat_add(p.cnt.stats, ST_TERM, c_term);
-	stat_add(p.cnt.stats, ST_DROPPED, c_drop); stat_add(p.cnt.stats, ST_EVENTS, c_events); stat_add(p.cnt.stats, ST_SHADOW, c_inline_shadow);
+	stat_add(p.cnt.stats, ST_DROPPED, c_drop); stat_add(p.cnt.stats, ST_EVENTS, c_events); stat_add(p.cnt.stats, ST_SHADOW, c_inline_shadow + c_hinted);
+	if (!EXACT) stat_add(p.cnt.stats, ST_HINTED, c_hinted);
 }
 template <bool COUNT>
 __global__ void __launch_bounds__(kTravBlock, 8) k_intersect_shadow(const Params p, const uint32_t bounce) {
@@ -779,7 +782,10 @@
 		},
 		[&](Walk& t, const float4* row) { return t.template step_staged<COUNT>(row, parent, &c_sphere, &c_box); },
 		[&](const Walk& t, uint32_t idx) {
-			if (t.occluded) return;
+			if (t.occluder != kNoNode) {
+				if (p.shadow_hint) p.shadow_hint[p.SK[idx]] = t.occluder;
+				return;
+			}
 			const f3 L{p.q.SL[idx], p.q.SL[p.q.cap + idx], p.q.SL[2u * p.q.cap + idx]};
 			rad_add(p.rad, p.frame.npix, pid, L, f3{0.0f, 0.0f, 0.0f}, true, false); c_events++;
 		});
diff --git a/cpu-raytracing-experiments_b200/csrc/b2r_shade.h b/cpu-raytracing-experiments_b200/csrc/b2r_shade.h
--- a/cpu-raytracing-experiments_b200/csrc/b2r_shade.h
+++ b/cpu-raytracing-experiments_b200/csrc/b2r_shade.h
@@ -27,7 +27,7 @@
 }
 B2R_HD float4 ld4(const float4* p) { return *p; }
 
-enum Stat { ST_EXT = 0, ST_SHADOW, ST_HITS, ST_TERM, ST_DROPPED, ST_SPHERE, ST_BOX, ST_EVENTS, ST_COUNT };
+enum Stat { ST_EXT = 0, ST_SHADOW, ST_HITS, ST_TERM, ST_DROPPED, ST_SPHERE, ST_BOX, ST_EVENTS, ST_HINTED, ST_COUNT };
 
 struct SceneDev {
 	const float4* prims;
@@ -97,6 +97,8 @@
 	float* rad;
 	float* acc;
 	const float4* mat_diel;
+	uint32_t* shadow_hint; uint32_t shadow_hint_mask;
+	uint32_t* SK;
 };
 
 B2R_HD void pixel_xy(uint32_t t, const FrameDev& fr, int32_t* x, int32_t* y) {
@@ -132,7 +134,7 @@
 	f3 P; TangentQuat T; float n_dot_v; f3 albedo; bool emissive; int32_t mat; float r2; f3 v_local; float alpha;
 	bool inside; float4 diel; f3 P_in;
 };
-struct ShadowRay { f3 o, d; float tfar; f3 L; };
+struct ShadowRay { f3 o, d; float tfar; f3 L; uint32_t pick; };
 
 B2R_HD bool dielectric_scatter(f3 v, float r, float u0, f3* dir, float* F) {
 	const float c = sel_min(sel_max(v.z, 0.0f), 1.0f);
@@ -207,8 +209,20 @@
 	const float w = power_heuristic_over_f(lpdf, bpdf);
 	rad = scale3(rad, w);
 	if (sel_max(sel_max(rad.x, rad.y), rad.z) <= 0.0f) return false;
-	out->o = sf.P; out->d = L; out->tfar = ldist; out->L = rad;
+	out->o = sf.P; out->d = L; out->tfar = ldist; out->L = rad; out->pick = pick;
 	return true;
+}
+B2R_HD uint32_t shadow_hint_key(int32_t prim, uint32_t pick, uint32_t mask) { return hash_u32(static_cast<uint32_t>(prim) * 0x9e3779b9u + pick) & mask; }
+B2R_HD bool shadow_hint_resolves(const SceneDev& sc, const uint32_t* table, uint32_t mask, int32_t prim, const ShadowRay& sr, uint32_t* key) {
+	*key = shadow_hint_key(prim, sr.pick, mask);
+#if defined(__CUDA_ARCH__)
+	uint32_t hint; asm("ld.relaxed.gpu.global.u32 %0, [%1];" : "=r"(hint) : "l"(table + *key));
+#else
+	const uint32_t hint = table[*key];
+#endif
+	if (hint >= sc.n_prims) return false;
+	const float4 sp = ld4(sc.prims + hint);
+	return sphere_hit_any(sp.x, sp.y, sp.z, sp.w, sr.o.x, sr.o.y, sr.o.z, sr.d.x, sr.d.y, sr.d.z, sr.tfar);
 }
 template <bool DIELECTRIC = false>
 B2R_HD f3 shade_emission(const SceneDev& sc, const Surface& sf, const PathState& s, float depth, uint32_t bounce, bool mis) {
@@ -378,11 +392,11 @@
 constexpr uint32_t kNoNode = 0xffffffffu;
 template <class Stack>
 struct TravAnyT : TravBase {
-	float tfar; bool occluded;
+	float tfar; uint32_t occluder;
 	uint32_t root, up, skip;
 	Stack stack;
 	B2R_HD void begin(const Ray& r, float limit, uint32_t start, const uint32_t* __restrict__ parent) {
-		arm(r); tfar = limit; occluded = false; stack.reset();
+		arm(r); tfar = limit; occluder = kNoNode; stack.reset();
 		node = root = start; up = start != 0u ? ldg_u32(parent + start) : 0u; skip = kNoNode;
 	}
 	template <bool COUNT, bool STAGED>
@@ -408,7 +422,7 @@
 			leaves &= leaves - 1u;
 			const float4 sp = node_f4<STAGED>(n, 2 * k);
 			if (COUNT) (*c_sphere)++;
-			if (sphere_hit_any(sp.x, sp.y, sp.z, sp.w, ox, oy, oz, dx, dy, dz, tfar)) { occluded = true; return false; }
+			if (sphere_hit_any(sp.x, sp.y, sp.z, sp.w, ox, oy, oz, dx, dy, dz, tfar)) { occluder = static_cast<uint32_t>(~as_int(node_f4<STAGED>(n, 2 * k + 1).z)); return false; }
 		}
 		if (next == kNoNode && (!stack.empty() || stack.refill())) next = stack.pop();
 		if (next == kNoNode && root != 0u) { skip = root; root = up; next = up; up = ldg_u32(parent + up); }
@@ -429,10 +443,12 @@
 	*best_out = t.best; *prim_out = t.prim;
 }
 template <bool COUNT>
-B2R_HD bool traverse_any(const WideNode* __restrict__ wide, const Ray& r, float tfar, uint32_t* c_sphere, uint32_t* c_box, const uint32_t* __restrict__ parent = nullptr, uint32_t start = 0u) {
+B2R_HD bool traverse_any(const WideNode* __restrict__ wide, const Ray& r, float tfar, uint32_t* c_sphere, uint32_t* c_box, const uint32_t* __restrict__ parent = nullptr, uint32_t start = 0u,
+                         uint32_t* occluder_out = nullptr) {
 	TravAny t; t.begin(r, tfar, start, parent);
 	while (t.template step<COUNT>(wide, parent, c_sphere, c_box)) {}
-	return t.occluded;
+	if (occluder_out) *occluder_out = t.occluder;
+	return t.occluder != kNoNode;
 }
 
 constexpr float kHitNoise = 1.5e-6f;
diff --git a/include/b2r.h b/include/b2r.h
--- a/include/b2r.h
+++ b/include/b2r.h
@@ -141,6 +141,7 @@
 int  b2r_read_wide_nodes(b2r_ctx* ctx, void* out_host, uint32_t* n_wide_nodes, uint32_t* max_stack);
 int  b2r_read_link_tables(b2r_ctx* ctx, uint32_t* parent_out, uint32_t* leaf_node_out);
 int  b2r_get_origin_box(b2r_ctx* ctx, float lo_hi_out[6]);
+int  b2r_fill_shadow_hints(b2r_ctx* ctx, const uint32_t* values, uint32_t n);
 
 int  b2r_write_hdr(const char* path, const float* rgba, uint32_t width, uint32_t height);
 
diff --git a/profiles/shadow_hint_stats.py b/profiles/shadow_hint_stats.py
--- /dev/null
+++ b/profiles/shadow_hint_stats.py
@@ -0,0 +1,38 @@
+#!/usr/bin/env python
+import ctypes as C
+import os
+import sys
+ROOT = os.path.dirname(os.path.dirname(os.path.abspath(__file__)))
+sys.path[:0] = [ROOT, os.path.join(ROOT, "cpu-raytracing-experiments_b200")]
+import numpy as np
+import b2r, scenes
+
+W, H, SAMPLES, MB = (int(a) for a in sys.argv[1:5]) if len(sys.argv) >= 5 else (480, 272, 8, 16)
+TABLES = [20, 22, 0]
+
+
+def main():
+    import __graft_entry__ as g
+    hc = C.CDLL(g.build_hostcheck())
+    ps = b2r.PreparedScene(scenes.random_scene(100000), W, H)
+    bits = np.array(TABLES, np.uint32); out = np.zeros((len(TABLES), MB, 4), np.uint64)
+    vp = lambda a: C.c_void_p(a.ctypes.data)
+    rc = hc.hc_shadow_hint_stats(vp(ps.prims), len(ps.prims), vp(ps.material), len(ps.material), vp(ps.lights), len(ps.lights), vp(ps.geometry), vp(ps.camera),
+                                 W, H, MB, 0, SAMPLES, vp(bits), len(TABLES), vp(out))
+    assert rc == 0, rc
+    print(f"C3 scene, {W}x{H}, samples 0..{SAMPLES - 1}, max_bounces {MB}, {len(ps.lights)} lights: per table, resolved rays / queued rays, "
+          f"and the walk visits of the resolved rays / all walk visits")
+    names = [f"2^{b}" if b else "collision-free" for b in TABLES]
+    print("bounce  rays      visits/ray  " + "  ".join(f"{n:>22s}" for n in names))
+    for b in range(MB - 1):
+        r = out[0, b]
+        if r[0] == 0:
+            continue
+        cols = "  ".join(f"{out[c, b, 1] / out[c, b, 0]:9.3f} / {out[c, b, 3] / out[c, b, 2]:9.3f}" for c in range(len(TABLES)))
+        print(f"{b:6d}  {int(r[0]):8d}  {r[2] / r[0]:10.2f}  {cols}")
+    tot = out.sum(axis=1)
+    print("all     " + f"{int(tot[0, 0]):8d}  {tot[0, 2] / tot[0, 0]:10.2f}  " + "  ".join(f"{tot[c, 1] / tot[c, 0]:9.3f} / {tot[c, 3] / tot[c, 2]:9.3f}" for c in range(len(TABLES))))
+
+
+if __name__ == "__main__":
+    main()
diff --git a/profiles/shadow_hint_workload.py b/profiles/shadow_hint_workload.py
--- /dev/null
+++ b/profiles/shadow_hint_workload.py
@@ -0,0 +1,80 @@
+#!/usr/bin/env python
+import json, os, subprocess, sys, time
+ROOT = os.path.dirname(os.path.dirname(os.path.abspath(__file__)))
+sys.path.insert(0, os.path.join(ROOT, "cpu-raytracing-experiments_b200"))
+import numpy as np
+import b2r, scenes
+
+W, H, MB, K, SPP = 1920, 1088, 16, 8, 16
+FRAMES = int(os.environ.get("FRAMES", "10"))
+OUT_DIR = sys.argv[1] if len(sys.argv) > 1 else "shadow_hint_workload_out"
+
+
+def card():
+    try:
+        q = subprocess.run(["nvidia-smi", "--query-gpu=name,power.limit", "--format=csv,noheader"], capture_output=True, text=True, timeout=30).stdout.strip()
+        return q.splitlines()[0]
+    except Exception as e:
+        return f"unknown ({e})"
+
+
+def renderer(ps, hints, flags=0):
+    if hints:
+        os.environ.pop("B2R_NO_SHADOW_HINT", None)
+    else:
+        os.environ["B2R_NO_SHADOW_HINT"] = "1"
+    try:
+        return b2r.Renderer(ps, W, H, max_bounces=MB, buckets=K, flags=flags)
+    finally:
+        os.environ.pop("B2R_NO_SHADOW_HINT", None)
+
+
+def frame_time(ps, hints):
+    r = renderer(ps, hints)
+    for _ in range(2):
+        r.ResetAccumulator(); r.Accumulate(SPP); r.RenderDevice()
+    r.sync(); r.reset_counters()
+    t0 = time.perf_counter()
+    for _ in range(FRAMES):
+        r.ResetAccumulator(); r.Accumulate(SPP); r.RenderDevice()
+    r.sync(); ms = (time.perf_counter() - t0) * 1e3 / FRAMES
+    cnt = r.counters()
+    paths, shadow = r.bounce_counts()
+    assert r.Render(); fb = r.framebuffer.copy(); r.close()
+    return dict(frame_ms=ms, shadow_rays=cnt["shadow_rays"] / FRAMES, hinted=cnt["shadow_hinted"] / FRAMES, extension_rays=cnt["extension_rays"] / FRAMES,
+                paths=paths.tolist(), shadow_queued=shadow.tolist()), fb
+
+
+def kernel_times(ps, hints):
+    r = renderer(ps, hints, b2r.FLAG_NO_GRAPH)
+    r.ResetAccumulator(); r.Accumulate(SPP); r.sync(); r.kernel_times(reset=True)
+    for _ in range(3):
+        r.ResetAccumulator(); r.Accumulate(SPP)
+    r.sync(); kt = r.kernel_times(reset=True); r.close()
+    return {k: v[0] / 3 for k, v in kt.items() if k in ("intersect_closest", "shade", "intersect_shadow")}
+
+
+def main():
+    os.makedirs(OUT_DIR, exist_ok=True)
+    info = card()
+    print(f"card: {info}; C3 {W}x{H} {SPP} spp K={K} mb={MB}, {FRAMES} frames per row")
+    ps = b2r.PreparedScene(scenes.random_scene(100000), W, H)
+    rows, fbs = [], {}
+    for hints in (True, False, True, False):
+        row, fb = frame_time(ps, hints)
+        row["hints"] = hints; rows.append(row); fbs[hints] = fb
+        print(json.dumps({k: v for k, v in row.items() if k not in ("paths", "shadow_queued")}))
+    identical = bool(np.array_equal(fbs[True].view(np.uint32), fbs[False].view(np.uint32)))
+    on, off = rows[0], rows[1]
+    per_bounce = [dict(bounce=b, queued_off=off["shadow_queued"][b], queued_on=on["shadow_queued"][b],
+                       resolved=(1.0 - on["shadow_queued"][b] / off["shadow_queued"][b]) if off["shadow_queued"][b] else 0.0) for b in range(MB - 1)]
+    for pb in per_bounce:
+        print(json.dumps(pb))
+    kt = {"on": kernel_times(ps, True), "off": kernel_times(ps, False)}
+    print(json.dumps(dict(kernel_ms_per_frame=kt, frames_identical=identical)))
+    json.dump(dict(card=info, frames=FRAMES, rows=rows, per_bounce=per_bounce, kernel_ms_per_frame=kt, frames_identical=identical),
+              open(os.path.join(OUT_DIR, "shadow_hint_workload.json"), "w"), indent=1)
+
+
+if __name__ == "__main__":
+    main()
```

Result: faster. 5948 (median of 6 runs) (+1.5%).
